# christopherkarani/Wax

Measured on NVIDIA H100. Metric: queries/sec cosine top-10 @ 10Mx384 fp32, higher is better.
Workload: dtype f32

## Files before the change

include/wax_vs_cuda.h:

```cpp
#ifndef WAX_VS_CUDA_H
#define WAX_VS_CUDA_H

#include <stddef.h>
#include <stdint.h>

#ifdef __cplusplus
extern "C" {
#endif

typedef struct wax_vs_engine wax_vs_engine;

enum {
    WAX_VS_OK = 0,
    WAX_VS_ERR_NULL = -1,
    WAX_VS_ERR_DIMENSION = -2,
    WAX_VS_ERR_CAPACITY = -3,
    WAX_VS_ERR_CUDA = -4,
    WAX_VS_ERR_FORMAT = -5,
    WAX_VS_ERR_ARGUMENT = -6,
    WAX_VS_ERR_BUFFER = -7,
    WAX_VS_ERR_UNSUPPORTED = -8
};

enum { WAX_VS_COSINE = 0, WAX_VS_DOT = 1, WAX_VS_L2 = 2 };
// ... 131 lines not shown
                             int64_t top_k, uint64_t row_offset, wax_vs_candidate *d_candidates,
                             void *cuda_stream);

int32_t wax_vs_search_batch_device(wax_vs_engine *engine, const float *d_queries, uint32_t n_queries,
                                   int64_t top_k, uint64_t row_offset, wax_vs_candidate *d_candidates,
                                   void *cuda_stream);

#define WAX_VS_SHARD_HANDLE_BYTES 128
#define WAX_VS_SHARD_MAX_RANKS 16
#define WAX_VS_SHARD_MAX_K 128
int32_t wax_vs_shard_open(wax_vs_engine *engine, int32_t rank, int32_t world, uint64_t row_offset,
                          uint8_t *out_handle );
int32_t wax_vs_shard_connect(wax_vs_engine *engine, const uint8_t *handles ,
                             int32_t n_handles);
int32_t wax_vs_shard_close(wax_vs_engine *engine);
int32_t wax_vs_shard_search(wax_vs_engine *engine, const float *query, uint32_t query_len, int64_t top_k,
                            uint64_t *out_ids, float *out_scores, uint32_t out_cap, uint32_t *out_n);
int32_t wax_vs_merge_candidates_device(wax_vs_engine *engine, const wax_vs_candidate *d_gathered, uint32_t world,
                                       uint32_t n_queries, uint32_t k, uint32_t k_out, wax_vs_candidate *d_out,
                                       void *cuda_stream);
int32_t wax_vs_shard_search_filtered(wax_vs_engine *engine, const float *query, uint32_t query_len, int64_t top_k,
                                     const uint64_t *frame_ids, uint64_t n_ids, int32_t mode, uint64_t *out_ids,
                                     float *out_scores, uint32_t out_cap, uint32_t *out_n);
int32_t wax_vs_shard_search_device(wax_vs_engine *engine, const float *d_query, int64_t top_k,
                                   wax_vs_candidate *d_candidates, void *cuda_stream);


int32_t wax_vs_serialized_length(wax_vs_engine *engine, uint64_t *out);
int32_t wax_vs_serialize(wax_vs_engine *engine, uint8_t *dst, uint64_t cap, uint64_t *out_len);
int32_t wax_vs_deserialize(wax_vs_engine *engine, const uint8_t *src, uint64_t len);

const char *wax_vs_last_error(void);


int32_t wax_vs_debug_pool_stats(wax_vs_engine *engine, uint64_t *allocations, uint64_t *reuses);

int32_t wax_vs_debug_fill_synthetic(wax_vs_engine *engine, uint64_t seed, uint64_t first_row,
                                    uint64_t rows, uint64_t id_base, int32_t normalize);
int32_t wax_vs_debug_read_rows(wax_vs_engine *engine, uint64_t first, uint64_t n, float *dst);

int32_t wax_vs_debug_time_search(wax_vs_engine *engine, uint32_t n_queries, int64_t top_k, uint64_t seed,
                                 uint32_t warmup, uint32_t iters, float *out_ms_total,
                                 uint64_t *out_launches);

int32_t wax_vs_debug_time_shard_search(wax_vs_engine *engine, uint32_t n_queries, int64_t top_k, uint64_t seed,
                                       uint32_t warmup, uint32_t iters, float *out_ms_total, uint64_t *out_launches);

int32_t wax_vs_debug_transfer_probe(wax_vs_engine *engine, uint64_t bytes, float *out7);

int32_t wax_vs_debug_phase_trace(wax_vs_engine *engine, int64_t top_k, uint32_t iters, float *out5);

int32_t wax_vs_debug_batch_stats(wax_vs_engine *engine, uint64_t *tensor_queries, uint64_t *fallback_queries);

int32_t wax_vs_debug_counter(wax_vs_engine *engine, const char *name, uint64_t *out);

int32_t wax_vs_debug_time_search_batch(wax_vs_engine *engine, uint32_t n_queries, int64_t top_k, uint64_t seed,
                                       uint32_t warmup, uint32_t iters, float *out_ms_total,
                                       uint64_t *out_launches, uint32_t *out_unproven);

int32_t wax_vs_debug_batch_nominations(wax_vs_engine *engine, const float *queries, uint32_t n_queries, int64_t top_k,
                                       const uint32_t *allow_bits, float *out_scores, uint32_t *out_ok,
                                       uint64_t *out_heaps, uint64_t heaps_cap, uint32_t *out_shape);

int32_t wax_vs_debug_shadow_nominations(wax_vs_engine *engine, const float *query, int64_t top_k, const uint32_t *allow_bits,
                                        uint64_t *out_keys, uint32_t *out_ok, wax_vs_candidate *out_result,
                                        uint32_t *out_shape);

int32_t wax_vs_debug_read_shadow(wax_vs_engine *engine, uint64_t first, uint64_t n, uint16_t *dst);

int32_t wax_vs_debug_int8_nominations(wax_vs_engine *engine, const float *query, int64_t top_k, const uint32_t *allow_bits,
                                      uint64_t *out_keys, uint32_t *out_ok, wax_vs_candidate *out_result,
                                      uint32_t *out_shape);

int32_t wax_vs_debug_read_int8_shadow(wax_vs_engine *engine, uint64_t first, uint64_t n, uint8_t *dst_codes,
                                      float *dst_scales, float *out_rho_max);

int32_t wax_vs_debug_u4_nominations(wax_vs_engine *engine, const float *query, int64_t top_k, const uint32_t *allow_bits,
                                    uint64_t *out_keys, uint64_t keys_cap, uint32_t *out_ok, wax_vs_candidate *out_result,
                                    uint32_t *out_shape, float *out_bound);

int32_t wax_vs_debug_read_u4_shadow(wax_vs_engine *engine, uint64_t first, uint64_t n, uint8_t *dst_codes,
                                    float *dst_half_steps, float *out_rho_max);

int32_t wax_vs_debug_stream_read(wax_vs_engine *engine, uint32_t iters, float *out_best_ms, uint64_t *out_bytes);

int32_t wax_vs_debug_set_option(wax_vs_engine *engine, const char *key, int64_t value);

const char *wax_vs_version(void);

#ifdef __cplusplus
}
#endif
#endif
```

wax_b200/_lib.py:

```python
from __future__ import annotations

import ctypes as C
from pathlib import Path

PKG = Path(__file__).resolve().parent
LIB_PATH = PKG / "libwaxvs_cuda.so"

OK, ERR_NULL, ERR_DIMENSION, ERR_CAPACITY, ERR_CUDA, ERR_FORMAT, ERR_ARGUMENT, ERR_BUFFER, ERR_UNSUPPORTED = (
    0, -1, -2, -3, -4, -5, -6, -7, -8)
MAX_RESULTS = 10_000
NO_FILTER = 0xFFFFFFFF
MAX_DIMENSIONS = 1_000_000
MAX_PER_GROUP = 128
SHARD_HANDLE_BYTES, SHARD_MAX_RANKS, SHARD_MAX_K = 128, 16, 128
INT64_MIN, INT64_MAX = -(1 << 63), (1 << 63) - 1


class Candidate(C.Structure):
    _fields_ = [("distance", C.c_float), ("valid", C.c_uint32), ("row", C.c_uint64), ("frame_id", C.c_uint64)]


class Where(C.Structure):
    _fields_ = [("after", C.c_int64), ("before", C.c_int64), ("all_tags", C.c_uint64), ("no_tags", C.c_uint64)]

# ... 18 lines not shown
    "wax_vs_remove": (C.c_int32, [_eng, C.c_uint64]),
    "wax_vs_remove_batch": (C.c_int32, [_eng, _u64p, C.c_uint64, _u64p]),
    "wax_vs_search": (C.c_int32, [_eng, _f32p, C.c_uint32, C.c_int64, _u64p, _f32p, C.c_uint32, _u32p]),
    "wax_vs_search_filtered": (C.c_int32, [_eng, _f32p, C.c_uint32, C.c_int64, _u64p, C.c_uint64, C.c_int32, _u64p, _f32p,
                                           C.c_uint32, _u32p]),
    "wax_vs_search_batch_filtered": (C.c_int32, [_eng, _f32p, C.c_uint32, C.c_uint32, C.c_int64, _u64p, C.c_uint64, C.c_int32,
                                                 _u64p, _f32p, C.c_uint32, _u32p]),
    "wax_vs_shard_search_filtered": (C.c_int32, [_eng, _f32p, C.c_uint32, C.c_int64, _u64p, C.c_uint64, C.c_int32, _u64p,
                                                 _f32p, C.c_uint32, _u32p]),
    "wax_vs_search_batch_multi_filtered": (C.c_int32, [_eng, _f32p, C.c_uint32, C.c_uint32, C.c_int64, _u64p, _u64p,
                                                       C.POINTER(C.c_int32), C.c_uint32, _u32p, _u64p, _f32p, C.c_uint32,
                                                       _u32p]),
    "wax_vs_set_groups": (C.c_int32, [_eng, _u64p, _u64p, C.c_uint64, _u64p]),
    "wax_vs_search_grouped": (C.c_int32, [_eng, _f32p, C.c_uint32, C.c_int64, C.c_uint32, _u64p, C.c_uint64, C.c_int32,
                                          _u64p, _f32p, _u64p, C.c_uint32, _u32p]),
    "wax_vs_search_batch_grouped": (C.c_int32, [_eng, _f32p, C.c_uint32, C.c_uint32, C.c_int64, C.c_uint32, _u64p,
                                                C.c_uint64, C.c_int32, _u64p, _f32p, _u64p, C.c_uint32, _u32p]),
    "wax_vs_set_attributes": (C.c_int32, [_eng, _u64p, C.POINTER(C.c_int64), _u64p, C.c_uint64, _u64p]),
    "wax_vs_search_batch_where": (C.c_int32, [_eng, _f32p, C.c_uint32, C.c_uint32, C.c_int64, _u64p, _u64p,
                                              C.POINTER(C.c_int32), C.c_uint32, _u32p, C.c_void_p, C.c_uint32, _u32p,
                                              _u64p, _f32p, C.c_uint32, _u32p]),
    "wax_vs_search_batch_grouped_where": (C.c_int32, [_eng, _f32p, C.c_uint32, C.c_uint32, C.c_int64, C.c_uint32, _u64p,
                                                      C.c_uint64, C.c_int32, C.c_void_p, _u64p, _f32p, _u64p, C.c_uint32,
                                                      _u32p]),
    "wax_vs_set_locations": (C.c_int32, [_eng, _u64p, _f64p, _f64p, C.c_uint64, _u64p]),
    "wax_vs_location_box": (C.c_int32, [C.c_double, C.c_double, C.c_double, C.POINTER(C.c_int32), C.POINTER(C.c_int32)]),
    "wax_vs_location_bin": (C.c_int32, [C.c_double, C.c_double, C.POINTER(C.c_int32), C.POINTER(C.c_int32)]),
    "wax_vs_search_batch_where_near": (C.c_int32, [_eng, _f32p, C.c_uint32, C.c_uint32, C.c_int64, _u64p, _u64p,
                                                   C.POINTER(C.c_int32), C.c_uint32, _u32p, C.c_void_p, C.c_uint32,
                                                   _u32p, _u64p, _f32p, C.c_uint32, _u32p]),
    "wax_vs_search_batch_grouped_where_near": (C.c_int32, [_eng, _f32p, C.c_uint32, C.c_uint32, C.c_int64, C.c_uint32,
                                                           _u64p, C.c_uint64, C.c_int32, C.c_void_p, _u64p, _f32p, _u64p,
                                                           C.c_uint32, _u32p]),
    "wax_vs_search_batch_grouped_multi_where": (C.c_int32, [_eng, _f32p, C.c_uint32, C.c_uint32, C.c_int64, C.c_uint32,
                                                            _u64p, _u64p, C.POINTER(C.c_int32), C.c_uint32, _u32p,
                                                            C.c_void_p, C.c_uint32, _u32p, _u64p, _f32p, _u64p,
                                                            C.c_uint32, _u32p]),
    "wax_vs_set_terms": (C.c_int32, [_eng, _u64p, _u64p, _u64p, C.c_uint64, _u64p]),
    "wax_vs_search_batch_where_terms": (C.c_int32, [_eng, _f32p, C.c_uint32, C.c_uint32, C.c_int64, _u64p, _u64p,
                                                    C.POINTER(C.c_int32), C.c_uint32, _u32p, C.c_void_p, C.c_uint32,
                                                    _u32p, _u64p, _u64p, _u64p, _f32p, C.c_uint32, _u32p]),
    "wax_vs_search_batch": (C.c_int32, [_eng, _f32p, C.c_uint32, C.c_uint32, C.c_int64, _u64p, _f32p,
                                        C.c_uint32, _u32p]),
    "wax_vs_search_device": (C.c_int32, [_eng, C.c_void_p, C.c_uint32, C.c_int64, C.c_uint64, C.c_void_p,
                                         C.c_void_p]),
    "wax_vs_search_batch_device": (C.c_int32, [_eng, C.c_void_p, C.c_uint32, C.c_int64, C.c_uint64, C.c_void_p,
                                               C.c_void_p]),
    "wax_vs_merge_candidates_device": (C.c_int32, [_eng, C.c_void_p, C.c_uint32, C.c_uint32, C.c_uint32, C.c_uint32,
                                                   C.c_void_p, C.c_void_p]),
    "wax_vs_shard_open": (C.c_int32, [_eng, C.c_int32, C.c_int32, C.c_uint64, _u8p]),
    "wax_vs_shard_connect": (C.c_int32, [_eng, _u8p, C.c_int32]),
    "wax_vs_shard_close": (C.c_int32, [_eng]),
    "wax_vs_shard_search": (C.c_int32, [_eng, _f32p, C.c_uint32, C.c_int64, _u64p, _f32p, C.c_uint32, _u32p]),
    "wax_vs_shard_search_device": (C.c_int32, [_eng, C.c_void_p, C.c_int64, C.c_void_p, C.c_void_p]),
    "wax_vs_serialized_length": (C.c_int32, [_eng, _u64p]),
    "wax_vs_serialize": (C.c_int32, [_eng, _u8p, C.c_uint64, _u64p]),
    "wax_vs_deserialize": (C.c_int32, [_eng, _u8p, C.c_uint64]),
    "wax_vs_last_error": (C.c_char_p, []),
    "wax_vs_debug_pool_stats": (C.c_int32, [_eng, _u64p, _u64p]),
    "wax_vs_debug_fill_synthetic": (C.c_int32, [_eng, C.c_uint64, C.c_uint64, C.c_uint64, C.c_uint64, C.c_int32]),
    "wax_vs_debug_read_rows": (C.c_int32, [_eng, C.c_uint64, C.c_uint64, _f32p]),
    "wax_vs_debug_time_search": (C.c_int32, [_eng, C.c_uint32, C.c_int64, C.c_uint64, C.c_uint32, C.c_uint32,
                                             _f32p, _u64p]),
    "wax_vs_debug_time_shard_search": (C.c_int32, [_eng, C.c_uint32, C.c_int64, C.c_uint64, C.c_uint32, C.c_uint32,
                                                   _f32p, _u64p]),
    "wax_vs_debug_transfer_probe": (C.c_int32, [_eng, C.c_uint64, _f32p]),
    "wax_vs_debug_phase_trace": (C.c_int32, [_eng, C.c_int64, C.c_uint32, _f32p]),
    "wax_vs_debug_batch_stats": (C.c_int32, [_eng, _u64p, _u64p]),
    "wax_vs_debug_counter": (C.c_int32, [_eng, C.c_char_p, _u64p]),
    "wax_vs_debug_time_search_batch": (C.c_int32, [_eng, C.c_uint32, C.c_int64, C.c_uint64, C.c_uint32, C.c_uint32,
                                                   _f32p, _u64p, _u32p]),
    "wax_vs_debug_batch_nominations": (C.c_int32, [_eng, _f32p, C.c_uint32, C.c_int64, _u32p, _f32p, _u32p, _u64p,
                                                   C.c_uint64, _u32p]),
    "wax_vs_debug_shadow_nominations": (C.c_int32, [_eng, _f32p, C.c_int64, _u32p, _u64p, _u32p, C.POINTER(Candidate),
                                                    _u32p]),
    "wax_vs_debug_read_shadow": (C.c_int32, [_eng, C.c_uint64, C.c_uint64, C.POINTER(C.c_uint16)]),
    "wax_vs_debug_int8_nominations": (C.c_int32, [_eng, _f32p, C.c_int64, _u32p, _u64p, _u32p, C.POINTER(Candidate),
                                                  _u32p]),
    "wax_vs_debug_read_int8_shadow": (C.c_int32, [_eng, C.c_uint64, C.c_uint64, _u8p, _f32p, _f32p]),
    "wax_vs_debug_u4_nominations": (C.c_int32, [_eng, _f32p, C.c_int64, _u32p, _u64p, C.c_uint64, _u32p,
                                                C.POINTER(Candidate), _u32p, _f32p]),
    "wax_vs_debug_read_u4_shadow": (C.c_int32, [_eng, C.c_uint64, C.c_uint64, _u8p, _f32p, _f32p]),
    "wax_vs_debug_stream_read": (C.c_int32, [_eng, C.c_uint32, _f32p, _u64p]),
    "wax_vs_debug_set_option": (C.c_int32, [_eng, C.c_char_p, C.c_int64]),
    "wax_vs_version": (C.c_char_p, []),
}

_lib = None


def lib() -> C.CDLL:
    global _lib
    if _lib is None:
        if not LIB_PATH.exists():
            raise ImportError(
                f"{LIB_PATH} is missing: the CUDA extension is the only implementation of the vector scan. "
                "Build it with `python -m wax_b200.build` (or __graft_entry__.build()).")
        handle = C.CDLL(str(LIB_PATH))
        for name, (restype, argtypes) in SIGNATURES.items():
            fn = getattr(handle, name)
            fn.restype = restype
            fn.argtypes = argtypes
        _lib = handle
    return _lib


def last_error() -> str:
    return lib().wax_vs_last_error().decode("utf-8", "replace")
```

wax_b200/csrc/waxvs_batch.cuh:

```cuda
#pragma once
#include <cuda.h>
#include <cuda_bf16.h>

#include "waxvs_common.cuh"
#include "waxvs_scan.cuh"

namespace waxvs {

constexpr int kBatchM = 128;
constexpr int kBatchN = 128;
constexpr int kBatchKBlock = 32;
constexpr int kBatchKBlockBf16 = 64;
constexpr int kBatchRescore = 256;
constexpr int kBatchRescoreMax = 1024;
constexpr uint32_t kBatchABytes = kBatchM * 128u;
constexpr uint32_t kBatchBBytes = kBatchN * 128u;
constexpr uint32_t kBatchStageBytes = kBatchABytes + kBatchBBytes;
constexpr int kBatchStageSlots = 8;
constexpr uint32_t kBatchScoreStride = kBatchN + 8;
constexpr uint32_t kBatchScoreBytes = kBatchM * kBatchScoreStride * 4u;
constexpr int kBatchMaxStages = 6;
constexpr uint32_t kBatchSmemOptin = 227u * 1024u;
__host__ __device__ constexpr uint32_t batch_smem_bytes(int stages, int heap, uint32_t ares_kb = 0) {
    return ares_kb * kBatchABytes + stages * (ares_kb ? kBatchBBytes : kBatchStageBytes) + kBatchScoreBytes +
// ... 141 lines not shown
                                                        float *inv_norm, uint32_t *max_norm_bits,
                                                        float *half_sq = nullptr) {
    const int lane = threadIdx.x & 31;
    const uint32_t warps = (gridDim.x * blockDim.x) >> 5;
    const bool vec4 = (dims % 4u) == 0u;
    float local_max = 0.0f;
    for (uint32_t row = (blockIdx.x * blockDim.x + threadIdx.x) >> 5; row < n_rows; row += warps) {
        const float *v = corpus + static_cast<size_t>(row) * dims;
        float b0 = 0.f, b1 = 0.f, b2 = 0.f, b3 = 0.f;
        if (vec4) {
            const float4 *v4 = reinterpret_cast<const float4 *>(v);
            for (uint32_t c = lane; c < dims / 4u; c += 32u) {
                const float4 x = __ldg(v4 + c);
                b0 = __fmaf_rn(x.x, x.x, b0); b1 = __fmaf_rn(x.y, x.y, b1);
                b2 = __fmaf_rn(x.z, x.z, b2); b3 = __fmaf_rn(x.w, x.w, b3);
            }
        } else {
            for (uint32_t base = 4u * lane; base < dims; base += 128u) {
                const float x = __ldg(v + base); b0 = __fmaf_rn(x, x, b0);
                if (base + 1 < dims) { const float y = __ldg(v + base + 1); b1 = __fmaf_rn(y, y, b1); }
                if (base + 2 < dims) { const float z = __ldg(v + base + 2); b2 = __fmaf_rn(z, z, b2); }
                if (base + 3 < dims) { const float w = __ldg(v + base + 3); b3 = __fmaf_rn(w, w, b3); }
            }
        }
        const float s = warp_butterfly_sum(__fadd_rn(__fadd_rn(b0, b1), __fadd_rn(b2, b3)));
        const float nrm = __fsqrt_rn(s);
        if (lane == 0) inv_norm[row] = (s == 0.0f) ? 0.0f : __fdiv_rn(1.0f, nrm);
        if constexpr (HALF_SQ) {
            if (lane == 0) half_sq[row] = 0.5f * s;
        }
        if (finite_f32(nrm)) {
            local_max = fmaxf(local_max, nrm);
        } else {
            float m = 0.0f;
            bool bad = false;
            for (uint32_t i = lane; i < dims; i += 32u) {
                const float x = __ldg(v + i);
                bad |= !finite_f32(x);
                m = fmaxf(m, fabsf(x));
            }
            if (!__any_sync(WAXVS_FULL_MASK, bad)) {
                for (int o = 16; o > 0; o >>= 1) m = fmaxf(m, __shfl_xor_sync(WAXVS_FULL_MASK, m, o));
                float t = 0.0f;
                for (uint32_t i = lane; i < dims; i += 32u) {
                    const float y = __fdiv_rn(__ldg(v + i), m);
                    t = __fmaf_rn(y, y, t);
                }
                local_max = fmaxf(local_max, m * __fsqrt_rn(warp_butterfly_sum(t)));
            }
        }
    }
    if (lane == 0 && local_max > 0.0f) atomicMax(max_norm_bits, __float_as_uint(local_max));
}

__global__ void __launch_bounds__(256) shadow_bf16_kernel(const float *__restrict__ src, const float *__restrict__ scale,
                                                          uint64_t n_rows, uint32_t dims, __nv_bfloat16 *__restrict__ dst) {
    const uint32_t d4 = dims >> 2;
    const uint64_t total = n_rows * d4;
    const float4 *s4 = reinterpret_cast<const float4 *>(src);
    uint2 *o = reinterpret_cast<uint2 *>(dst);
    for (uint64_t i = static_cast<uint64_t>(blockIdx.x) * blockDim.x + threadIdx.x; i < total;
         i += static_cast<uint64_t>(gridDim.x) * blockDim.x) {
        float4 x = __ldcs(s4 + i);
        if (scale) {
            const float w = __ldg(scale + i / d4);
            x.x *= w; x.y *= w; x.z *= w; x.w *= w;
        }
        const __nv_bfloat162 lo = __floats2bfloat162_rn(x.x, x.y), hi = __floats2bfloat162_rn(x.z, x.w);
        uint2 v;
        v.x = *reinterpret_cast<const uint32_t *>(&lo);
        v.y = *reinterpret_cast<const uint32_t *>(&hi);
        auto clamp_half = [](uint32_t h, float src) -> uint32_t {
            return ((h & 0x7FFFu) == 0x7F80u && finite_f32(src)) ? ((h & 0x8000u) | 0x7F7Fu) : h;
        };
        v.x = clamp_half(v.x & 0xFFFFu, x.x) | (clamp_half(v.x >> 16, x.y) << 16);
        v.y = clamp_half(v.y & 0xFFFFu, x.z) | (clamp_half(v.y >> 16, x.w) << 16);
        o[i] = v;
    }
}

constexpr uint32_t kInt8MaxChunks = 12;
__global__ void __launch_bounds__(256) shadow_int8_kernel(const float *__restrict__ src, const float *__restrict__ scale_in,
                                                          uint64_t n_rows, uint32_t dims, uint32_t *__restrict__ dst,
                                                          float *__restrict__ scale, uint32_t *rho_max_bits) {
    const int lane = threadIdx.x & 31;
    const uint64_t warps = (static_cast<uint64_t>(gridDim.x) * blockDim.x) >> 5;
    const uint32_t d4 = dims >> 2, cn = d4 / 32u;
    uint32_t local_max = 0;
    for (uint64_t row = (static_cast<uint64_t>(blockIdx.x) * blockDim.x + threadIdx.x) >> 5; row < n_rows; row += warps) {
        const float4 *v4 = reinterpret_cast<const float4 *>(src) + row * d4;
        const float w = scale_in ? __ldg(scale_in + row) : 1.0f;
        float4 x[kInt8MaxChunks];
        float m = 0.0f;
        bool bad = false;
#pragma unroll
        for (uint32_t c = 0; c < kInt8MaxChunks; ++c) {
            if (c >= cn) break;
            x[c] = __ldcs(v4 + lane + 32u * c);
            if (scale_in) { x[c].x *= w; x[c].y *= w; x[c].z *= w; x[c].w *= w; }
            bad |= !finite_f32(x[c].x) || !finite_f32(x[c].y) || !finite_f32(x[c].z) || !finite_f32(x[c].w);
            m = fmaxf(m, fmaxf(fmaxf(fabsf(x[c].x), fabsf(x[c].y)), fmaxf(fabsf(x[c].z), fabsf(x[c].w))));
        }
        for (int o = 16; o > 0; o >>= 1) m = fmaxf(m, __shfl_xor_sync(WAXVS_FULL_MASK, m, o));
        bad = __any_sync(WAXVS_FULL_MASK, bad);
        const float s = __fdiv_rn(m, 127.0f);
        double r2 = 0.0;
#pragma unroll
        for (uint32_t c = 0; c < kInt8MaxChunks; ++c) {
            if (c >= cn) break;
            const float xs[4] = {x[c].x, x[c].y, x[c].z, x[c].w};
            uint32_t packed = 0;
#pragma unroll
            for (int j = 0; j < 4; ++j) {
                int code = 0;
                if (s > 0.0f && !bad) code = max(-127, min(127, __float2int_rn(__fdiv_rn(xs[j], s))));
                packed |= static_cast<uint32_t>(code + 128) << (8 * j);
                const double e = static_cast<double>(xs[j]) - static_cast<double>(s) * static_cast<double>(code);
                r2 = fma(e, e, r2);
            }
            dst[row * d4 + lane + 32u * c] = packed;
        }
        for (int o = 16; o > 0; o >>= 1) r2 += __shfl_xor_sync(WAXVS_FULL_MASK, r2, o);
        float rho = __double2float_ru(sqrt(r2) * (1.0 + 0x1p-40));
        if (bad || !finite_f32(s) || !finite_f32(rho)) rho = INFINITY;
        if (lane == 0) scale[row] = s;
        local_max = max(local_max, __float_as_uint(rho));
    }
    if (lane == 0 && local_max) atomicMax(rho_max_bits, local_max);
}

__global__ void __launch_bounds__(256) shadow_u4_kernel(const float *__restrict__ src, const float *__restrict__ scale_in,
                                                        uint64_t n_rows, uint32_t dims, uint32_t *__restrict__ dst,
                                                        float *__restrict__ half_step, uint32_t *rho_max_bits) {
    const int lane = threadIdx.x & 31;
    const uint64_t warps = (static_cast<uint64_t>(gridDim.x) * blockDim.x) >> 5;
    const uint32_t d4 = dims >> 2, cn = d4 / 32u;
    uint32_t local_max = 0;
    for (uint64_t row = (static_cast<uint64_t>(blockIdx.x) * blockDim.x + threadIdx.x) >> 5; row < n_rows; row += warps) {
        const float4 *v4 = reinterpret_cast<const float4 *>(src) + row * d4;
        const float w = scale_in ? __ldg(scale_in + row) : 1.0f;
        float4 x[kInt8MaxChunks];
        float m = 0.0f;
        bool bad = false;
#pragma unroll
        for (uint32_t c = 0; c < kInt8MaxChunks; ++c) {
            if (c >= cn) break;
            x[c] = __ldcs(v4 + lane + 32u * c);
            if (scale_in) { x[c].x *= w; x[c].y *= w; x[c].z *= w; x[c].w *= w; }
            bad |= !finite_f32(x[c].x) || !finite_f32(x[c].y) || !finite_f32(x[c].z) || !finite_f32(x[c].w);
            m = fmaxf(m, fmaxf(fmaxf(fabsf(x[c].x), fabsf(x[c].y)), fmaxf(fabsf(x[c].z), fabsf(x[c].w))));
        }
        for (int o = 16; o > 0; o >>= 1) m = fmaxf(m, __shfl_xor_sync(WAXVS_FULL_MASK, m, o));
        bad = __any_sync(WAXVS_FULL_MASK, bad);
        const float h = __fdiv_rn(m, 16.0f), step = __fmul_rn(2.0f, h);
        double r2 = 0.0;
#pragma unroll
        for (uint32_t c = 0; c < kInt8MaxChunks; ++c) {
            if (c >= cn) break;
            const float xs[4] = {x[c].x, x[c].y, x[c].z, x[c].w};
            uint32_t nibbles = 0;
#pragma unroll
            for (int j = 0; j < 4; ++j) {
                int u = 8;
                if (h > 0.0f && !bad) u = max(0, min(15, __float2int_rd(__fdiv_rn(xs[j], step)) + 8));
                nibbles |= static_cast<uint32_t>(u) << (8 * j);
                const double e = static_cast<double>(xs[j]) - static_cast<double>(h) * static_cast<double>(2 * u - 15);
                r2 = fma(e, e, r2);
            }
            const uint32_t high = __shfl_down_sync(WAXVS_FULL_MASK, nibbles, 1);
            if ((lane & 1) == 0) dst[row * (d4 / 2u) + (lane >> 1) + 16u * c] = nibbles | (high << 4);
        }
        for (int o = 16; o > 0; o >>= 1) r2 += __shfl_xor_sync(WAXVS_FULL_MASK, r2, o);
        float rho = __double2float_ru(sqrt(r2) * (1.0 + 0x1p-40));
        if (bad || !finite_f32(h) || !finite_f32(rho)) rho = INFINITY;
        if (lane == 0) half_step[row] = h;
        local_max = max(local_max, __float_as_uint(rho));
    }
    if (lane == 0 && local_max) atomicMax(rho_max_bits, local_max);
}

template <bool BF16, bool FILTER, bool ARES, bool PAIR, bool DUMP = false, bool L2 = false>
__global__ void __launch_bounds__(kBatchThreads, 1)
batch_nominate_kernel(const __grid_constant__ CUtensorMap tmap_q, const __grid_constant__ CUtensorMap tmap_c,
                      const BatchParams p) {
    extern __shared__ uint8_t smem_raw[];
    uint8_t *smem = smem_raw + ((1024u - (smem_u32(smem_raw) & 1023u)) & 1023u);
    constexpr uint32_t KB_ELEMS = BF16 ? kBatchKBlockBf16 : kBatchKBlock;
    constexpr uint32_t STAGE_BYTES = ARES ? kBatchBBytes : kBatchStageBytes;
    constexpr uint32_t B_OFF = ARES ? 0u : kBatchABytes;
    const uint32_t num_kb = p.dims / KB_ELEMS;
    const uint32_t nst = p.stages, heap_n = p.kprime;
    const uint32_t ares_bytes = ARES ? num_kb * kBatchABytes : 0u;
    uint8_t *a_res = smem;
    uint8_t *stages = smem + ares_bytes;
    float *score = reinterpret_cast<float *>(stages + nst * STAGE_BYTES);
    float *scale_smem = score + kBatchM * kBatchScoreStride;
    uint64_t *full = reinterpret_cast<uint64_t *>(scale_smem + kBatchN);
    uint64_t *empty = full + kBatchMaxStages;
    uint64_t *a_full = empty + kBatchMaxStages;
    uint64_t *stage_smem = reinterpret_cast<uint64_t *>(reinterpret_cast<uint8_t *>(full) + 256);
    uint64_t *heap_smem = stage_smem + kBatchStageSlots * kBatchM;

    const int warp = threadIdx.x >> 5, lane = threadIdx.x & 31;
    const uint32_t rank = PAIR ? cluster_ctarank() : 0u;
    const uint32_t unit = PAIR ? blockIdx.x / 2u : blockIdx.x;
    const uint32_t units_per_slice = PAIR ? p.groups / 2u : p.groups;
    const uint32_t group = PAIR ? (unit % units_per_slice) * 2u + rank : unit % units_per_slice;
    const uint32_t slice = unit / units_per_slice;
    const uint32_t tile_lo = static_cast<uint32_t>(static_cast<uint64_t>(p.tiles_total) * slice / p.slices);
    const uint32_t tile_hi = static_cast<uint32_t>(static_cast<uint64_t>(p.tiles_total) * (slice + 1) / p.slices);

    if (warp == 4 && lane == 0) {
        tma_prefetch_desc(&tmap_q);
        tma_prefetch_desc(&tmap_c);
        for (int s = 0; s < kBatchMaxStages; ++s) { mbar_init(&full[s], 1); mbar_init(&empty[s], PAIR ? 8 : 4); }
        mbar_init(a_full, 1);
        mbar_fence_init();
    }
    if (PAIR) cluster_sync_all(); else __syncthreads();

    if (warp == 4) {
        if (lane == 0) {
            if (ARES && tile_lo < tile_hi) {
                mbar_arrive_expect_tx(a_full, ares_bytes);
                for (uint32_t kb = 0; kb < num_kb; ++kb)
                    tma_load_2d(a_res + kb * kBatchABytes, &tmap_q, a_full, static_cast<int32_t>(kb * KB_ELEMS),
                                static_cast<int32_t>(group * kBatchM));
            }
            uint32_t stage = 0, phase = 0;
            for (uint32_t tile = tile_lo; tile < tile_hi; ++tile) {
                for (uint32_t kb = 0; kb < num_kb; ++kb) {
                    mbar_wait_parity(&empty[stage], phase ^ 1u);
                    uint8_t *a = stages + stage * STAGE_BYTES;
                    mbar_arrive_expect_tx(&full[stage], STAGE_BYTES);
                    if (!ARES)
                        tma_load_2d(a, &tmap_q, &full[stage], static_cast<int32_t>(kb * KB_ELEMS), static_cast<int32_t>(group * kBatchM));
                    if (PAIR)
                        tma_load_2d_multicast(a + B_OFF + rank * (kBatchBBytes / 2), &tmap_c, &full[stage],
                                              static_cast<int32_t>(kb * KB_ELEMS),
                                              static_cast<int32_t>(tile * kBatchN + rank * (kBatchN / 2)), 0x3);
                    else
                        tma_load_2d(a + B_OFF, &tmap_c, &full[stage], static_cast<int32_t>(kb * KB_ELEMS),
                                    static_cast<int32_t>(tile * kBatchN));
                    if (++stage == nst) { stage = 0; phase ^= 1u; }
                }
            }
        }
        __syncwarp();
        if (PAIR) cluster_sync_all();
        return;
    }

    const uint32_t tid = threadIdx.x;
    const uint32_t q = group * kBatchM + tid;
    const bool q_valid = q < p.n_queries && !p.no_insert;
    const uint32_t *allow = p.allow_bits;
    if (p.query_filter && q < p.n_queries) {
        const uint32_t f = __ldg(p.query_filter + q);
// ... 694 lines not shown
```

wax_b200/csrc/waxvs_engine.cu:

```cuda
#include <cuda_runtime.h>

#include <algorithm>
#include <atomic>
#include <cstdarg>
#include <cstdio>
#include <cstring>
#include <mutex>
#include <new>
#include <shared_mutex>
#include <string>
#include <unordered_map>
#include <chrono>
#include <random>
#include <thread>
#include <unistd.h>
#include <cmath>
#include <vector>

#include "../../include/wax_vs_cuda.h"
#include "waxvs_common.cuh"
#include "waxvs_scan.cuh"
#include "waxvs_select.cuh"
#include "waxvs_synth.cuh"
#include "waxvs_batch.cuh"
// ... 132 lines not shown
    int batch_retry = 1;
    int filter_bf16 = 1;
    int filter_cap = 8192;
    int inline_query = 1;
    int host_delivery = 1;
    int tail_select = 1;
    int shard_fused = 1;
    int batch_l2 = 0;
    int single_shadow = 0;
    uint64_t filter_bitset_bytes = 2ull << 30;
    int shadow_scan = 1;
    uint64_t shadow_scan_min_bytes = 512ull << 20;
    int shadow_rows_per_step = 0, shadow_warps = 0, shadow_stages = 0;
    uint64_t int8_scan_min_bytes = 512ull << 20;
    int int8_rows_per_step = 0, int8_warps = 0, int8_stages = 0;
    uint64_t u4_scan_min_bytes = 2048ull << 20;
    int u4_rows_per_step = 0, u4_warps = 0, u4_stages = 0;
};

struct SearchCtx {
    cudaStream_t stream = nullptr;
    bool own_stream = false;
    DevBuf<float> d_queries;
    DevBuf<wax_vs_candidate> d_out;
    PinnedBuf<float> h_queries;
    PinnedBuf<wax_vs_candidate> h_out;
    DevBuf<uint64_t> d_block_keys;
    DevBuf<uint32_t> d_ticket;
    DevBuf<uint32_t> d_dist_keys;
    DevBuf<SelectState> d_select;
    DevBuf<uint64_t> d_sel_keys;
    cudaEvent_t ev0 = nullptr, ev1 = nullptr;
    DevBuf<uint64_t> d_heaps;
    DevBuf<uint32_t> d_ok;
    PinnedBuf<uint32_t> h_ok;
    DevBuf<uint32_t> d_tau;
    DevBuf<__nv_bfloat16> d_queries_bf16;
    DevBuf<float> d_retry_q;
    DevBuf<wax_vs_candidate> d_retry_out;
    DevBuf<uint32_t> d_retry_ok;
    DevBuf<float> d_tau_star;
    PinnedBuf<float> h_tau_star;
    DevBuf<float> d_filter_tau;
    PinnedBuf<float> h_filter_tau;
    DevBuf<uint32_t> d_cand_count;
    DevBuf<uint32_t> d_cand_rows;
    DevBuf<uint64_t> d_cand_keys;
    DevBuf<uint32_t> d_mask;
    DevBuf<uint32_t> d_filter_rows;
    DevBuf<uint64_t> d_filter_spec;
    DevBuf<uint32_t> d_query_filter;
    DevBuf<uint32_t> d_retry_filter;
    DevBuf<uint2> d_gather_span;
    DevBuf<uint64_t> d_gather_keys;
    DevBuf<wax_vs_candidate> d_shard_local;
    DevBuf<unsigned long long> d_group_best;
    DevBuf<uint32_t> d_group_keys;
    DevBuf<uint2> d_group_spans;
    PinnedBuf<uint2> h_group_spans;
    DevBuf<ExpandItem> d_expand_items;
    DevBuf<uint64_t> d_expand[3];
    PinnedBuf<uint64_t> h_expand;
    DevBuf<uint64_t> d_bg_keys;
    PinnedBuf<uint64_t> h_bg_keys;
    DevBuf<uint32_t> d_bg_status;
    PinnedBuf<uint32_t> h_bg_status;
    DevBuf<CoverExpand> d_bg_expand;
    PinnedBuf<CoverExpand> h_bg_expand;
    DevBuf<ScoreItem> d_score_items;
    PinnedBuf<unsigned long long> h_flag;
    unsigned long long host_seq = 0;
    DevBuf<WhereNearItem> d_where_items;
    DevBuf<uint32_t> d_where_counts;
    DevBuf<uint64_t> d_term_ids;
    DevBuf<TermSpan> d_term_spans;
    DevBuf<TermUnit> d_term_units;
    DevBuf<uint32_t> d_term_counts;
    DevBuf<uint32_t> d_term_deny;
    DevBuf<uint32_t> d_proof_count;
    PinnedBuf<uint32_t> h_proof_count;
    uint32_t seen_failed = 0;
    bool last_u4 = false;
    DevBuf<uint32_t> d_u4_aux;
    ~SearchCtx() {
        if (ev0) cudaEventDestroy(ev0);
        if (ev1) cudaEventDestroy(ev1);
        if (own_stream && stream) cudaStreamDestroy(stream);
    }
};

struct wax_vs_engine {
    int device = 0;
    int sm_count = 132;
    size_t smem_optin = 0;
    uint32_t dims = 0;
    uint8_t similarity = 0;

    float *d_corpus = nullptr;
    uint64_t cap_rows = 0, n_rows = 0;

    bool ids_identity = true;
    uint64_t id_base = 0;
    std::vector<uint64_t> ids;
    IdMap map;
    bool map_valid = true;
    bool ids_sorted = true;
    DevBuf<uint64_t> d_ids;
    bool d_ids_dirty = true;
    std::mutex ids_mu;

    std::shared_mutex rw;
    std::mutex pool_mu;
    std::vector<SearchCtx *> pool;
    std::unordered_map<void *, SearchCtx *> stream_ctx;
    uint64_t pool_allocs = 0, pool_reuses = 0;
    Tuning tune;

    DevBuf<float> d_inv_norm;
    DevBuf<uint32_t> d_max_norm;
    DevBuf<float> d_half_sq;
    uint64_t norms_rows = 0;
    std::mutex norms_mu;
    DevBuf<__nv_bfloat16> d_shadow;
    uint64_t shadow_rows = 0;
    bool shadow_valid = false, shadow_unavailable = false;
    struct CodedShadow {
        uint32_t bits = 8;
        DevBuf<uint32_t> codes;
        DevBuf<float> scale;
        DevBuf<uint32_t> rho;
        uint64_t rows = 0;
        bool valid = false, unavailable = false;
        bool coarse = false;
        float rho_max = 0.0f, eps_rel = INFINITY;
        void release() { codes.release(); scale.release(); rows = 0; valid = false; }
        void invalidate(uint64_t keep_prefix) {
            rows = std::min(rows, keep_prefix);
            valid = false;
            if (keep_prefix == 0) coarse = false;
        }
    } i8, u4{4};
    uint32_t u4_demoted = 0, u4_demote_window = 16;
    bool u4_probing = false;
    uint64_t single_int8_queries = 0;
    uint64_t single_u4_queries = 0;
    uint64_t batch_tensor_queries = 0, batch_fallback_queries = 0;
    uint64_t batch_bf16_queries = 0, batch_retry_queries = 0, batch_tf32_queries = 0, batch_filter_bf16_queries = 0;
    uint64_t filter_bitset_passes = 0;
    bool groups_set = false;
    std::vector<uint64_t> groups;
    struct GroupIndex {
        DevBuf<uint32_t> perm, row_group, starts;
        uint32_t n_groups = 0;
        bool valid = false;
    } gindex;
    std::mutex group_mu;
    uint64_t group_index_builds = 0;
    bool attrs_set = false;
    std::vector<AttrRow> attrs;
    DevBuf<AttrRow> d_attrs;
    bool attrs_dev_valid = false;
    std::mutex attrs_mu;
    uint64_t attribute_uploads = 0;
    bool locs_set = false;
    std::vector<LocRow> locs;
    DevBuf<LocRow> d_locs;
    bool locs_dev_valid = false;
    uint64_t location_uploads = 0;
    struct TermRef {
        uint64_t off;
        uint32_t n;
    };
    bool terms_set = false;
    std::vector<TermRef> term_refs;
    std::vector<uint64_t> term_pool;
    uint64_t term_garbage = 0;
    struct TermIndex {
        DevBuf<uint64_t> keys, start;
        DevBuf<uint32_t> postings;
        uint32_t n_terms = 0;
        uint64_t n_postings = 0;
        bool valid = false;
    } tindex;
    std::mutex term_mu;
    uint64_t term_index_builds = 0;
    uint64_t grouped_batch_covered_queries = 0, grouped_batch_expanded_groups = 0, grouped_batch_fallback_queries = 0;
    uint64_t grouped_batch_expansion_passes = 0;
    uint32_t bf16_skip_batches = 0;
    uint32_t shadow_scan_skip = 0;
    uint32_t heap_bump = 0, heap_bump_ttl = 0, heap_backoff = 256;
    bool heap_probing = false;
    uint32_t last_heap = 0;
    struct Ingest {
        cudaStream_t stream = nullptr;
        cudaEvent_t ev[2] = {nullptr, nullptr};
        uint8_t *pin[2] = {nullptr, nullptr};
        size_t pin_bytes = 0;
        DevBuf<float> d_stage;
        DevBuf<uint32_t> d_index;
        int threads = 1;
        ~Ingest() {
            for (int i = 0; i < 2; ++i) {
                if (pin[i]) cudaFreeHost(pin[i]);
                if (ev[i]) cudaEventDestroy(ev[i]);
            }
            if (stream) cudaStreamDestroy(stream);
        }
    } ing;
    uint64_t ingest_h2d_bytes = 0, ingest_d2h_bytes = 0;
    std::mutex ingest_mu;
    std::mutex attr_mu;
    std::unordered_map<const void *, int> smem_granted;
    std::atomic<bool> async_pending{false};
    unsigned long long *debug_trace = nullptr;

    struct Shard {
        bool open = false, connected = false;
        int rank = 0, world = 0;
// ... 329 lines not shown
    int32_t rc = c->d_select.ensure(1, "selection state");
    if (!rc) rc = c->d_sel_keys.ensure(16384, "selected keys");
    if (rc) return rc;
    const int sgrid = std::max(1, std::min<int>(e->sm_count * 4, static_cast<int>((n + 511) / 512)));
    select_init_kernel<<<1, 256, 0, stream>>>(c->d_select, k);
    for (int pass = 0; pass < kSelectPasses; ++pass) {
        select_hist_kernel<<<sgrid, 512, 0, stream>>>(keys, n, c->d_select, pass);
        select_scan_kernel<<<1, 1024, 0, stream>>>(c->d_select, pass);
    }
    select_compact_kernel<<<sgrid, 512, 0, stream>>>(keys, n, c->d_select, c->d_sel_keys, 16384);
    uint32_t pow2 = 64;
    while (pow2 < k) pow2 <<= 1;
    CUDA_TRY(grant_smem(e, select_sort_kernel, pow2 * sizeof(uint64_t)));
    select_sort_kernel<<<1, 1024, pow2 * sizeof(uint64_t), stream>>>(c->d_select, c->d_sel_keys, pow2, p);
    CUDA_TRY(cudaGetLastError());
    *launches += 3 + 2 * kSelectPasses;
    return WAX_VS_OK;
}

static int tma_grid(const wax_vs_engine *e, const SearchCtx *c, const TmaConfig &cfg, ScanParams &p) {
    p.stages = static_cast<uint32_t>(cfg.stages);
    const uint64_t steps = (e->n_rows + cfg.R - 1) / cfg.R;
    const int max_grid = e->tune.grid > 0 ? e->tune.grid : e->sm_count;
    int grid = static_cast<int>(std::min<uint64_t>(max_grid, (steps + cfg.warps - 1) / cfg.warps));
    grid = std::max(std::min(grid, static_cast<int>(c->d_block_keys.cap / 128)), 1);
    if (e->tune.chunk_steps < 0)
        p.chunk_steps = static_cast<uint32_t>(std::max<uint64_t>(1, std::min<uint64_t>(8, steps / (static_cast<uint64_t>(grid) * cfg.warps * 2))));
    return grid;
}

static bool batch_bf16_wanted(const wax_vs_engine *e);
static int32_t ensure_shadow(wax_vs_engine *e, cudaStream_t stream);
static int32_t ensure_coded_shadow(wax_vs_engine *e, wax_vs_engine::CodedShadow &cs, cudaStream_t stream, bool keep_coarse = false);

constexpr uint32_t kShadowNominees = 128;
constexpr uint32_t kShadowRescore = 256;
constexpr uint32_t kShadowSkipQueries = 16;
static bool shadow_route_applies(const wax_vs_engine *e) {
    return e->tune.shadow_scan && (e->similarity == WAX_VS_COSINE || e->similarity == WAX_VS_DOT) && !e->debug_trace &&
           e->tune.batch_bf16 != 0 && e->dims % kBatchKBlockBf16 == 0 &&
           e->n_rows * e->dims * sizeof(float) >= e->tune.shadow_scan_min_bytes;
}
static int32_t int8_route_selected(wax_vs_engine *e, cudaStream_t stream, bool *use) {
    *use = false;
    TmaConfig cfg{};
    if (e->n_rows * e->dims * sizeof(float) < e->tune.int8_scan_min_bytes || !pick_tma_config(e, &cfg, 1, 1)) return WAX_VS_OK;
    const int32_t rc = ensure_coded_shadow(e, e->i8, stream);
    if (rc) return rc;
    *use = e->i8.valid && e->i8.eps_rel <= kBf16Eps;
    return WAX_VS_OK;
}
enum class RouteForm { kBf16, kInt8, kU4 };
static int32_t select_route_form(wax_vs_engine *e, cudaStream_t stream, bool demoted, RouteForm *form) {
    *form = RouteForm::kBf16;
    TmaConfig cfg{};
    int32_t rc;
    if (!demoted && e->n_rows * e->dims * sizeof(float) >= e->tune.u4_scan_min_bytes && pick_u4_config(e, &cfg)) {
        if ((rc = ensure_coded_shadow(e, e->u4, stream))) return rc;
        if (e->u4.valid && std::isfinite(e->u4.eps_rel)) { *form = RouteForm::kU4; return WAX_VS_OK; }
    }
    bool int8 = false;
    if ((rc = int8_route_selected(e, stream, &int8))) return rc;
    if (int8) *form = RouteForm::kInt8;
    return WAX_VS_OK;
}

static int32_t enqueue_shadow_nominations(wax_vs_engine *e, SearchCtx *c, const ScanParams &p, const TmaConfig &cfg,
                                          cudaStream_t stream, uint64_t *launches, uint32_t *shape = nullptr,
                                          RouteForm form = RouteForm::kBf16) {
    const bool int8 = form == RouteForm::kInt8, u4 = form == RouteForm::kU4;
    int32_t rc;
    if (u4 && !c->d_u4_aux) {
        if ((rc = c->d_u4_aux.ensure(3, "4-bit route state"))) return rc;
        CUDA_TRY(cudaMemsetAsync(c->d_u4_aux, 0xFF, 3 * sizeof(uint32_t), stream));
    }
    const size_t u4_keys = static_cast<size_t>(std::max(e->tune.grid, e->sm_count)) * kU4CtaNominees;
    if ((rc = c->d_heaps.ensure(std::max(static_cast<size_t>(kShadowNominees) * kNomineeStride, u4 ? u4_keys : 0), "nominee keys")) ||
        (rc = c->d_ok.ensure(1, "proof flags")) || (!p.query && (rc = c->d_queries.ensure(e->dims, "query buffer"))))
        return rc;

    ScanParams sp = p;
    sp.corpus = u4 ? reinterpret_cast<const float *>(e->u4.codes.p)
                   : int8 ? reinterpret_cast<const float *>(e->i8.codes.p) : reinterpret_cast<const float *>(e->d_shadow.p);
    sp.row_scale = u4 ? e->u4.scale.p : int8 ? e->i8.scale.p : nullptr;
    sp.u4_aux = u4 ? c->d_u4_aux.p : nullptr;
    sp.k = kShadowNominees;
    sp.out = nullptr; sp.host_out = nullptr; sp.host_flag = nullptr;
    sp.nominees = c->d_heaps;
    sp.query_store = p.query ? nullptr : c->d_queries.p;
    sp.tail_select = e->tune.tail_select ? 1u : 0u;
    sp.tail_smem_bytes = static_cast<uint32_t>(static_cast<size_t>(cfg.warps) * cfg.stages * cfg.R * e->dims *
                                               (int8 ? 1 : sizeof(__nv_bfloat16)));
    const int grid = tma_grid(e, c, cfg, sp);
    if (u4) CUDA_TRY(launch_u4_scan(e, sp, grid, cfg, stream));
    else if (int8) CUDA_TRY(launch_int8_scan(e, sp, grid, cfg, e->similarity, stream));
    else CUDA_TRY(launch_shadow_scan(e, sp, grid, cfg, e->similarity, stream));

    if (u4) {
        RescoreParams rp{};
        rp.corpus = e->d_corpus; rp.query = p.query ? p.query : c->d_queries.p;
        rp.dims = e->dims; rp.k = p.k; rp.n_nominees = static_cast<uint32_t>(grid) * kU4CtaNominees;
        rp.nominees = c->d_heaps; rp.aux = c->d_u4_aux; rp.max_norm_bits = e->d_max_norm; rp.rho_max = e->u4.rho_max;
        rp.block_keys = c->d_block_keys; rp.ticket = c->d_ticket; rp.work_counter = sp.work_counter; rp.out = p.out; rp.ok = c->d_ok;
        rp.frame_ids = p.frame_ids; rp.id_base = p.id_base; rp.row_offset = p.row_offset;
        rp.tail_smem_bytes = static_cast<uint32_t>(grid) * p.k * sizeof(uint64_t);
        if (rp.tail_smem_bytes > 48u * 1024u) rp.tail_smem_bytes = 0;
        const auto kernel = e->similarity == WAX_VS_COSINE ? shadow_rescore_kernel<kCosine> : shadow_rescore_kernel<kDot>;
        kernel<<<grid, 512, rp.tail_smem_bytes, stream>>>(rp);
        CUDA_TRY(cudaGetLastError());
    } else {
    FinishParams fp{};
    fp.corpus = e->d_corpus; fp.queries = p.query ? p.query : c->d_queries.p;
    fp.n_rows = p.n_rows; fp.dims = e->dims; fp.n_queries = 1; fp.groups = 1; fp.slices = 1;
    fp.kprime = kShadowNominees; fp.k = p.k; fp.metric = e->similarity;
    fp.heaps = c->d_heaps; fp.max_norm_bits = e->d_max_norm;
    fp.out = p.out; fp.ok = c->d_ok;
    fp.frame_ids = p.frame_ids; fp.id_base = p.id_base; fp.row_offset = p.row_offset;
    fp.pow2_all = 512; fp.rescore = kShadowRescore; fp.eps_rel = int8 ? e->i8.eps_rel : kBf16Eps;
    const size_t fsmem = static_cast<size_t>(fp.pow2_all + fp.rescore) * sizeof(uint64_t);
    const auto kernel = e->similarity == WAX_VS_COSINE ? batch_finish_kernel<kCosine> : batch_finish_kernel<kDot>;
    CUDA_TRY(grant_smem(e, kernel, fsmem));
    kernel<<<1, 512, fsmem, stream>>>(fp);
    CUDA_TRY(cudaGetLastError());
    }
    *launches += 2;
    if (shape) {
        const uint32_t s[7] = {static_cast<uint32_t>(cfg.C), static_cast<uint32_t>(cfg.R), static_cast<uint32_t>(cfg.warps),
                               static_cast<uint32_t>(cfg.stages), static_cast<uint32_t>(grid), sp.chunk_steps, sp.tail_select};
        std::copy(s, s + 7, shape);
    }
    return WAX_VS_OK;
}

static int32_t enqueue_shadow_route(wax_vs_engine *e, SearchCtx *c, ScanParams &p, cudaStream_t stream, uint64_t *launches) {
    if (!shadow_route_applies(e)) return WAX_VS_OK;
    TmaConfig cfg{};
    if (!pick_tma_config(e, &cfg, 1, sizeof(__nv_bfloat16))) return WAX_VS_OK;
    int32_t rc;
    if (!c->h_proof_count) {
        if ((rc = c->d_proof_count.ensure(2, "proof counts")) || (rc = c->h_proof_count.ensure(2, "proof count mirror"))) return rc;
        CUDA_TRY(cudaMemsetAsync(c->d_proof_count, 0, 2 * sizeof(uint32_t), stream));
        c->h_proof_count[0] = c->h_proof_count[1] = 0;
        c->seen_failed = 0;
    }
    bool demoted;
    {
        std::lock_guard<std::mutex> pg(e->pool_mu);
        const uint32_t failed = *static_cast<volatile uint32_t *>(c->h_proof_count + 1);
        if (failed != c->seen_failed) {
            c->seen_failed = failed;
            if (c->last_u4) {
                if (e->u4_probing) e->u4_demote_window = std::min(e->u4_demote_window * 2, 1u << 20);
                e->u4_demoted = e->u4_demote_window;
            } else {
                e->shadow_scan_skip = kShadowSkipQueries;
            }
        } else if (c->last_u4 && e->u4_probing) {
            e->u4_demote_window = 16;
        }
        if (c->last_u4) e->u4_probing = false;
        c->last_u4 = false;
        if (e->shadow_scan_skip > 0) { --e->shadow_scan_skip; return WAX_VS_OK; }
        demoted = e->u4_demoted > 0;
        if (demoted && --e->u4_demoted == 0) e->u4_probing = true;
    }
    RouteForm form;
    if ((rc = select_route_form(e, stream, demoted, &form))) return rc;
    if (form == RouteForm::kU4) {
        if (!pick_u4_config(e, &cfg)) return WAX_VS_OK;
    } else if (form == RouteForm::kInt8) {
        if (!pick_tma_config(e, &cfg, 1, 1)) return WAX_VS_OK;
    } else {
        if ((rc = ensure_shadow(e, stream))) return rc;
        if (!e->shadow_valid) return WAX_VS_OK;
    }
    if ((rc = enqueue_shadow_nominations(e, c, p, cfg, stream, launches, nullptr, form))) return rc;
    c->last_u4 = form == RouteForm::kU4;
    if (form != RouteForm::kBf16) {
        std::lock_guard<std::mutex> pg(e->pool_mu);
        ++(form == RouteForm::kU4 ? e->single_u4_queries : e->single_int8_queries);
    }
    p.proof_ok = c->d_ok;
    p.proof_count = c->d_proof_count;
    p.proof_count_host = c->h_proof_count;
    return WAX_VS_OK;
}

static ScanParams scan_params(const wax_vs_engine *e, SearchCtx *c, const float *d_query, uint32_t k_eff, uint64_t row_offset,
                              wax_vs_candidate *d_out, const uint64_t *d_ids, const uint32_t *d_mask) {
    ScanParams p{};
    p.corpus = e->d_corpus; p.query = d_query;
    p.n_rows = static_cast<uint32_t>(e->n_rows); p.dims = e->dims; p.k = k_eff;
// ... 153 lines not shown
        e->norms_rows = 0;
        const size_t want = static_cast<size_t>(std::max<uint64_t>(e->cap_rows, std::max<uint64_t>(e->n_rows, 1)));
        int32_t rc = e->d_inv_norm.ensure(want, "row norms");
        if (!rc && l2) rc = e->d_half_sq.ensure(want, "row half squared norms");
        if (rc) return rc;
    }
    if (!e->d_max_norm) {
        int32_t rc = e->d_max_norm.ensure(1, "max row norm");
        if (rc) return rc;
        e->norms_rows = 0;
    }
    if (e->norms_rows > e->n_rows) e->norms_rows = 0;
    if (e->norms_rows == 0) CUDA_TRY(cudaMemsetAsync(e->d_max_norm, 0, sizeof(uint32_t), stream));
    const uint64_t first = e->norms_rows, count = e->n_rows - first;
    if (count) {
        const int grid = static_cast<int>(std::min<uint64_t>(static_cast<uint64_t>(e->sm_count) * 8, (count + 7) / 8));
        if (l2)
            row_norms_kernel<true><<<std::max(grid, 1), 256, 0, stream>>>(e->d_corpus + first * e->dims, static_cast<uint32_t>(count),
                                                                          e->dims, e->d_inv_norm + first, e->d_max_norm,
                                                                          e->d_half_sq + first);
        else
            row_norms_kernel<<<std::max(grid, 1), 256, 0, stream>>>(e->d_corpus + first * e->dims, static_cast<uint32_t>(count), e->dims,
                                                                    e->d_inv_norm + first, e->d_max_norm);
        CUDA_TRY(cudaGetLastError());
    }
    CUDA_TRY(cudaStreamSynchronize(stream));
    e->norms_rows = e->n_rows;
    return WAX_VS_OK;
}
static int32_t ensure_norms(wax_vs_engine *e, cudaStream_t stream) {
    std::lock_guard<std::mutex> g(e->norms_mu);
    return ensure_norms_locked(e, stream);
}

static bool batch_bf16_wanted(const wax_vs_engine *e) {
    return e->tune.batch_bf16 != 0 && e->dims % kBatchKBlockBf16 == 0 && !e->shadow_unavailable;
}

static int32_t ensure_shadow(wax_vs_engine *e, cudaStream_t stream) {
    std::lock_guard<std::mutex> g(e->norms_mu);
    if ((e->shadow_valid && e->shadow_rows == e->n_rows) || e->shadow_unavailable) return WAX_VS_OK;
    int32_t rc = ensure_norms_locked(e, stream);
    if (rc) return rc;
    const size_t need = static_cast<size_t>(e->n_rows) * e->dims;
    const size_t pref = static_cast<size_t>(std::max<uint64_t>(e->cap_rows, e->n_rows)) * e->dims;
    if (e->d_shadow.cap < need) {
        e->d_shadow.release();
        e->shadow_rows = 0; e->shadow_valid = false;
        size_t free_b = 0, total_b = 0;
        size_t want = pref;
        size_t bytes = want * sizeof(__nv_bfloat16);
        const bool info = cudaMemGetInfo(&free_b, &total_b) == cudaSuccess;
        const size_t headroom = std::max<size_t>(size_t(2) << 30, total_b / 10);
        if (info && free_b < bytes + headroom) { want = need; bytes = want * sizeof(__nv_bfloat16); }
        if (!info || free_b < bytes + headroom || cudaMalloc(&e->d_shadow.p, bytes) != cudaSuccess) {
            cudaGetLastError();
            e->shadow_unavailable = true;
            return WAX_VS_OK;
        }
        e->d_shadow.cap = want;
    }
    if (e->shadow_rows > e->n_rows) e->shadow_rows = 0;
    const uint64_t first = e->shadow_rows, count = e->n_rows - first;
    if (count) {
        const int grid = static_cast<int>(std::min<uint64_t>(static_cast<uint64_t>(e->sm_count) * 16, (count * (e->dims / 4) + 255) / 256));
        shadow_bf16_kernel<<<std::max(grid, 1), 256, 0, stream>>>(e->d_corpus + first * e->dims,
                                                                  e->similarity == WAX_VS_COSINE ? e->d_inv_norm + first : nullptr,
                                                                  count, e->dims, e->d_shadow + first * e->dims);
        CUDA_TRY(cudaGetLastError());
    }
    CUDA_TRY(cudaStreamSynchronize(stream));
    e->shadow_rows = e->n_rows;
    e->shadow_valid = true;
    return WAX_VS_OK;
}

static int32_t ensure_coded_shadow(wax_vs_engine *e, wax_vs_engine::CodedShadow &cs, cudaStream_t stream, bool keep_coarse) {
    std::lock_guard<std::mutex> g(e->norms_mu);
    if ((cs.valid && cs.rows == e->n_rows) || cs.unavailable || (cs.coarse && !keep_coarse))
        return WAX_VS_OK;
    int32_t rc = ensure_norms_locked(e, stream);
    if (rc) return rc;
    if ((rc = cs.rho.ensure(1, "coded shadow bound"))) return rc;
    const size_t words = e->dims * cs.bits / 32;
    const uint64_t need = e->n_rows, pref = std::max<uint64_t>(e->cap_rows, e->n_rows);
    auto scale_entries = [](uint64_t rows) { return static_cast<size_t>((rows + 15) / 16 * 16); };
    if (cs.codes.cap < need * words || cs.scale.cap < scale_entries(need)) {
        cs.release();
        size_t free_b = 0, total_b = 0;
        uint64_t want = pref;
        auto bytes_for = [&](uint64_t rows) { return rows * words * sizeof(uint32_t) + scale_entries(rows) * sizeof(float); };
        const bool info = cudaMemGetInfo(&free_b, &total_b) == cudaSuccess;
        const size_t headroom = std::max<size_t>(size_t(2) << 30, total_b / 10);
        size_t reserve = 0;
        if (batch_bf16_wanted(e) && e->d_shadow.cap < static_cast<size_t>(need) * e->dims) {
            const size_t b_need = static_cast<size_t>(need) * e->dims * sizeof(__nv_bfloat16);
            const size_t b_pref = static_cast<size_t>(pref) * e->dims * sizeof(__nv_bfloat16);
            reserve = free_b >= b_pref + headroom ? b_pref : (free_b >= b_need + headroom ? b_need : 0);
        }
        if (info && free_b < bytes_for(want) + reserve + headroom) want = need;
        if (!info || free_b < bytes_for(want) + reserve + headroom ||
            cudaMalloc(&cs.codes.p, want * words * sizeof(uint32_t)) != cudaSuccess ||
            cudaMalloc(&cs.scale.p, scale_entries(want) * sizeof(float)) != cudaSuccess) {
            cudaGetLastError();
            cs.release();
            cs.unavailable = true;
            return WAX_VS_OK;
        }
        cs.codes.cap = want * words;
        cs.scale.cap = scale_entries(want);
        CUDA_TRY(cudaMemsetAsync(cs.scale, 0, scale_entries(want) * sizeof(float), stream));
    }
    if (cs.rows > e->n_rows) cs.rows = 0;
    if (cs.rows == 0) CUDA_TRY(cudaMemsetAsync(cs.rho, 0, sizeof(uint32_t), stream));
    const uint64_t first = cs.rows, count = e->n_rows - first;
    if (count) {
        const int grid = static_cast<int>(std::min<uint64_t>(static_cast<uint64_t>(e->sm_count) * 8, (count + 7) / 8));
        (cs.bits == 4 ? shadow_u4_kernel : shadow_int8_kernel)<<<std::max(grid, 1), 256, 0, stream>>>(
            e->d_corpus + first * e->dims, e->similarity == WAX_VS_COSINE ? e->d_inv_norm + first : nullptr, count, e->dims,
            cs.codes + first * words, cs.scale + first, cs.rho);
        CUDA_TRY(cudaGetLastError());
    }
    uint32_t bits[2] = {0, 0};
    CUDA_TRY(cudaMemcpyAsync(&bits[0], cs.rho, sizeof(uint32_t), cudaMemcpyDeviceToHost, stream));
    CUDA_TRY(cudaMemcpyAsync(&bits[1], e->d_max_norm, sizeof(uint32_t), cudaMemcpyDeviceToHost, stream));
    CUDA_TRY(cudaStreamSynchronize(stream));
    float rho, m;
    memcpy(&rho, &bits[0], sizeof rho);
    memcpy(&m, &bits[1], sizeof m);
    if (e->similarity == WAX_VS_COSINE) m = 1.0f;
    const float q = rho / m;
    cs.rho_max = rho;
    cs.eps_rel = (std::isfinite(q) && std::isfinite(m) && m > 0.0f)
                          ? (static_cast<double>(q) * m >= rho ? q : std::nextafter(q, INFINITY)) : INFINITY;
    cs.rows = e->n_rows;
    cs.valid = true;
    if (cs.bits == 4 ? !std::isfinite(cs.eps_rel) : cs.eps_rel > kBf16Eps) {
        cs.coarse = true;
        if (!keep_coarse) {
            cs.release();
        }
    }
    return WAX_VS_OK;
}

template <bool BF, bool FI, bool AR, bool PR, bool DUMP, bool L2>
static cudaError_t launch_nominate_inst(wax_vs_engine *e, uint32_t grid, uint32_t smem, cudaStream_t stream,
                                        const CUtensorMap &map_q, const CUtensorMap &map_c, const BatchParams &bp) {
    const auto kernel = batch_nominate_kernel<BF, FI, AR, PR, DUMP, L2>;
    const cudaError_t err = grant_smem(e, kernel, smem);
    if (err != cudaSuccess) return err;
    cudaLaunchConfig_t cfg{};
    cfg.gridDim = dim3(grid); cfg.blockDim = dim3(kBatchThreads); cfg.stream = stream; cfg.dynamicSmemBytes = smem;
    cudaLaunchAttribute attr[1];
    if (PR) {
        attr[0].id = cudaLaunchAttributeClusterDimension;
        attr[0].val.clusterDim.x = 2; attr[0].val.clusterDim.y = 1; attr[0].val.clusterDim.z = 1;
        cfg.attrs = attr; cfg.numAttrs = 1;
    }
    return cudaLaunchKernelEx(&cfg, kernel, map_q, map_c, bp);
}

template <bool DUMP, bool L2>
static cudaError_t launch_nominate_forms(wax_vs_engine *e, bool bf16, bool filter, bool ares, bool pair, uint32_t grid,
                                         uint32_t smem, cudaStream_t stream, const CUtensorMap &map_q,
                                         const CUtensorMap &map_c, const BatchParams &bp) {
#define WAXVS_NOM(BF, FI, AR, PR) return launch_nominate_inst<BF, FI, AR, PR, DUMP, L2>(e, grid, smem, stream, map_q, map_c, bp)
    if constexpr (!DUMP) {
        if (filter) {
            if (!bf16) WAXVS_NOM(false, true, false, false);
            if (ares) WAXVS_NOM(true, true, true, false);
            WAXVS_NOM(true, true, false, false);
        }
    }
    if (!bf16) {
        if (pair) WAXVS_NOM(false, false, false, true);
        WAXVS_NOM(false, false, false, false);
    }
    if (ares) {
        if (pair) WAXVS_NOM(true, false, true, true);
        WAXVS_NOM(true, false, true, false);
    }
    if (pair) WAXVS_NOM(true, false, false, true);
    WAXVS_NOM(true, false, false, false);
#undef WAXVS_NOM
}
template <bool DUMP>
static cudaError_t launch_nominate(wax_vs_engine *e, bool l2, bool bf16, bool filter, bool ares, bool pair, uint32_t grid,
                                   uint32_t smem, cudaStream_t stream, const CUtensorMap &map_q, const CUtensorMap &map_c,
                                   const BatchParams &bp) {
    return l2 ? launch_nominate_forms<DUMP, true>(e, bf16, filter, ares, pair, grid, smem, stream, map_q, map_c, bp)
              : launch_nominate_forms<DUMP, false>(e, bf16, filter, ares, pair, grid, smem, stream, map_q, map_c, bp);
}

static double poisson_tail(double m, int h) {
    double term = std::exp(-m);
    for (int i = 1; i <= h; ++i) term *= m / i;
    double tail = 0.0, t = term;
    for (int i = h + 1; i < h + 200 && t > 1e-300; ++i) { tail += t; t *= m / i; }
    return std::min(1.0, tail + t);
}

static uint32_t pick_heap(wax_vs_engine *e, bool bf16, uint32_t nq, uint32_t slices, uint32_t k_eff) {
// ... 2993 lines not shown
}

int32_t wax_vs_debug_time_search(wax_vs_engine *e, uint32_t n_queries, int64_t top_k, uint64_t seed,
                                 uint32_t warmup, uint32_t iters, float *out_ms_total, uint64_t *out_launches) {
    if (!e || !out_ms_total) return fail(WAX_VS_ERR_NULL, "NULL argument");
    if (n_queries == 0) n_queries = 1;
    std::shared_lock<std::shared_mutex> r(e->rw);
    DeviceGuard g(e->device);
    CtxLease lease(e);
    int32_t rc = lease.acquire();
    if (rc) return rc;
    SearchCtx *c = lease.c;
    const uint32_t k_eff = clamp_topk(top_k);
    const size_t qfloats = static_cast<size_t>(n_queries) * e->dims;
    if ((rc = c->d_queries.ensure(qfloats, "query buffer"))) return rc;
    if ((rc = c->d_out.ensure(static_cast<size_t>(n_queries) * k_eff, "result buffer"))) return rc;
    synth_fill_kernel<<<(n_queries + 255) / 256, 256, 0, c->stream>>>(c->d_queries, n_queries, e->dims, seed, 0, 1);
    CUDA_TRY(cudaGetLastError());
    uint64_t launches = 0;
    CtxLease lease2(e);
    if (e->tune.time_overlap) {
        if ((rc = lease2.acquire())) return rc;
        if ((rc = lease2.c->d_out.ensure(static_cast<size_t>(n_queries) * k_eff, "result buffer"))) return rc;
    }
    SearchCtx *c2 = lease2.c;
    if (shadow_route_applies(e)) {
        RouteForm form;
        if ((rc = select_route_form(e, c->stream, false, &form))) return rc;
        if (form == RouteForm::kBf16 && (rc = ensure_shadow(e, c->stream))) return rc;
    }
    for (uint32_t it = 0; it < warmup + iters; ++it) {
        if (it == warmup) {
            launches = 0;
            if (c2) { CUDA_TRY(cudaEventRecord(c2->ev0, c2->stream)); CUDA_TRY(cudaStreamWaitEvent(c->stream, c2->ev0, 0)); }
            CUDA_TRY(cudaEventRecord(c->ev0, c->stream));
            if (c2) CUDA_TRY(cudaStreamWaitEvent(c2->stream, c->ev0, 0));
        }
        const uint32_t qi = it % n_queries;
        SearchCtx *cc = (c2 && (it & 1u)) ? c2 : c;
        if (c2 && it == 0) { CUDA_TRY(cudaEventRecord(c->ev1, c->stream)); CUDA_TRY(cudaStreamWaitEvent(c2->stream, c->ev1, 0)); }
        rc = enqueue_search(e, cc, c->d_queries + static_cast<size_t>(qi) * e->dims, k_eff, 0,
                            cc->d_out + static_cast<size_t>(qi) * k_eff, nullptr, cc->stream, &launches, nullptr, nullptr,
                            nullptr, false, true);
        if (rc) { cudaStreamSynchronize(c->stream); if (c2) cudaStreamSynchronize(c2->stream); return rc; }
    }
    if (c2) { CUDA_TRY(cudaEventRecord(c2->ev1, c2->stream)); CUDA_TRY(cudaStreamWaitEvent(c->stream, c2->ev1, 0)); }
    CUDA_TRY(cudaEventRecord(c->ev1, c->stream));
    CUDA_TRY(cudaStreamSynchronize(c->stream));
    CUDA_TRY(cudaEventElapsedTime(out_ms_total, c->ev0, c->ev1));
    if (out_launches) *out_launches = launches;
    return WAX_VS_OK;
}

int32_t wax_vs_debug_stream_read(wax_vs_engine *e, uint32_t iters, float *out_best_ms, uint64_t *out_bytes) {
    if (!e || !out_best_ms || !out_bytes) return fail(WAX_VS_ERR_NULL, "NULL argument");
    std::shared_lock<std::shared_mutex> r(e->rw);
    DeviceGuard g(e->device);
    CtxLease lease(e);
    int32_t rc = lease.acquire();
    if (rc) return rc;
    SearchCtx *c = lease.c;
    const uint64_t bytes = e->n_rows * e->dims * sizeof(float) / 16 * 16;
    *out_bytes = bytes;
    *out_best_ms = 0.0f;
    if (bytes == 0) return WAX_VS_OK;
    float best = 1e30f;
    for (uint32_t it = 0; it < iters + 2; ++it) {
        CUDA_TRY(cudaEventRecord(c->ev0, c->stream));
        stream_read_kernel<<<e->sm_count * 4, 512, 0, c->stream>>>(reinterpret_cast<const uint4 *>(e->d_corpus),
                                                                     bytes / 16, c->d_ticket + 2);
        CUDA_TRY(cudaGetLastError());
        CUDA_TRY(cudaEventRecord(c->ev1, c->stream));
        CUDA_TRY(cudaStreamSynchronize(c->stream));
        float ms = 0;
        CUDA_TRY(cudaEventElapsedTime(&ms, c->ev0, c->ev1));
        if (it >= 2 && ms < best) best = ms;
    }
    CUDA_TRY(cudaMemsetAsync(c->d_ticket, 0, 4 * sizeof(uint32_t), c->stream));
    CUDA_TRY(cudaStreamSynchronize(c->stream));
    *out_best_ms = best;
    return WAX_VS_OK;
}

int32_t wax_vs_debug_transfer_probe(wax_vs_engine *e, uint64_t bytes, float *out7) {
    if (!e || !out7) return fail(WAX_VS_ERR_NULL, "NULL argument");
    std::unique_lock<std::shared_mutex> w(e->rw);
    DeviceGuard g(e->device);
    bytes = std::max<uint64_t>(bytes, 1u << 20);
    int32_t rc = ingest_staging(e, bytes);
    if (rc) return rc;
    auto &ig = e->ing;
    if ((rc = ig.d_stage.ensure(static_cast<size_t>((bytes + 3) / 4), "probe buffer"))) return rc;
    std::vector<uint8_t> host(bytes, 1);
    auto secs = [](auto t0) { return std::chrono::duration<double>(std::chrono::steady_clock::now() - t0).count(); };
    uint8_t *probe_pin = nullptr;
    {
        std::lock_guard<std::mutex> pool(g_staging_mu);
        if ((rc = shared_staging())) return rc;
        probe_pin = g_staging[0];
    }
    const size_t chunk = std::min<size_t>(kStagingBytes, bytes);
    auto best = [&](auto fn) { double b = 1e30; for (int i = 0; i < 3; ++i) { auto t0 = std::chrono::steady_clock::now(); fn(); b = std::min(b, secs(t0)); } return b; };
    out7[0] = static_cast<float>(chunk / 1e9 / best([&] { memcpy(probe_pin, host.data(), chunk); }));
    out7[1] = static_cast<float>(chunk / 1e9 / best([&] { parallel_memcpy(probe_pin, host.data(), chunk, ig.threads); }));
    out7[2] = static_cast<float>(chunk / 1e9 / best([&] { cudaMemcpyAsync(ig.d_stage, probe_pin, chunk, cudaMemcpyHostToDevice, ig.stream); cudaStreamSynchronize(ig.stream); }));
    out7[3] = static_cast<float>(chunk / 1e9 / best([&] { cudaMemcpyAsync(probe_pin, ig.d_stage, chunk, cudaMemcpyDeviceToHost, ig.stream); cudaStreamSynchronize(ig.stream); }));
    out7[4] = static_cast<float>(bytes / 1e9 / best([&] { upload_bytes(e, ig.d_stage, host.data(), bytes); }));
    out7[5] = static_cast<float>(bytes / 1e9 / best([&] { download_bytes(e, host.data(), ig.d_stage, bytes); }));
    out7[6] = static_cast<float>(ig.threads);
    CUDA_TRY(cudaGetLastError());
    return WAX_VS_OK;
}

int32_t wax_vs_debug_phase_trace(wax_vs_engine *e, int64_t top_k, uint32_t iters, float *out5) {
    if (!e || !out5) return fail(WAX_VS_ERR_NULL, "NULL argument");
    std::unique_lock<std::shared_mutex> w(e->rw);
    DeviceGuard g(e->device);
    CtxLease lease(e, true);
    int32_t rc = lease.acquire();
    if (rc) return rc;
    SearchCtx *c = lease.c;
    const uint32_t k_eff = clamp_topk(top_k);
    if ((rc = c->d_queries.ensure(static_cast<size_t>(e->dims), "query buffer"))) return rc;
    if ((rc = c->d_out.ensure(static_cast<size_t>(k_eff), "result buffer"))) return rc;
    synth_fill_kernel<<<1, 256, 0, c->stream>>>(c->d_queries, 1, e->dims, 99, 0, 1);
    unsigned long long *d_trace = nullptr;
    CUDA_TRY(cudaMalloc(&d_trace, 8 * sizeof(unsigned long long)));
    double acc[5] = {0, 0, 0, 0, 0};
    uint64_t launches = 0;
    for (uint32_t it = 0; it < iters + 3; ++it) {
        const unsigned long long init[8] = {~0ull, 0, 0, 0, 0, 0, 0, 0};
        cudaMemcpyAsync(d_trace, init, sizeof init, cudaMemcpyHostToDevice, c->stream);
        cudaStreamSynchronize(c->stream);
        e->debug_trace = d_trace;
        cudaEventRecord(c->ev0, c->stream);
        rc = enqueue_search(e, c, c->d_queries, k_eff, 0, c->d_out, nullptr, c->stream, &launches);
        cudaEventRecord(c->ev1, c->stream);
        e->debug_trace = nullptr;
        if (rc) { cudaStreamSynchronize(c->stream); cudaFree(d_trace); return rc; }
        unsigned long long t[8];
        cudaMemcpyAsync(t, d_trace, sizeof t, cudaMemcpyDeviceToHost, c->stream);
        cudaStreamSynchronize(c->stream);
        float ms = 0;
        cudaEventElapsedTime(&ms, c->ev0, c->ev1);
        if (it < 3) continue;
        for (int i = 0; i < 4; ++i) acc[i] += (t[i + 1] > t[0] && t[0] != ~0ull) ? (t[i + 1] - t[0]) * 1e-3 : 0.0;
        acc[4] += ms * 1e3;
    }
    cudaFree(d_trace);
    for (int i = 0; i < 5; ++i) out5[i] = static_cast<float>(acc[i] / std::max(iters, 1u));
    CUDA_TRY(cudaGetLastError());
    return WAX_VS_OK;
}

int32_t wax_vs_debug_batch_stats(wax_vs_engine *e, uint64_t *tensor_queries, uint64_t *fallback_queries) {
    if (!e) return fail(WAX_VS_ERR_NULL, "engine is NULL");
    std::lock_guard<std::mutex> g(e->pool_mu);
    if (tensor_queries) *tensor_queries = e->batch_tensor_queries;
    if (fallback_queries) *fallback_queries = e->batch_fallback_queries;
    return WAX_VS_OK;
}

int32_t wax_vs_debug_counter(wax_vs_engine *e, const char *name, uint64_t *out) {
    if (!e || !name || !out) return fail(WAX_VS_ERR_NULL, "NULL argument");
    std::lock_guard<std::mutex> g(e->pool_mu);
    if (!strcmp(name, "batch_tensor_queries")) *out = e->batch_tensor_queries;
// ... 142 lines not shown
                                       uint32_t *out_shape, RouteForm form, uint64_t keys_cap = 0, float *out_bound = nullptr) {
    const bool u4 = form == RouteForm::kU4, int8 = form != RouteForm::kBf16;
    if (!e || !query || !out_keys || !out_ok || !out_result || !out_shape || (u4 && !out_bound))
        return fail(WAX_VS_ERR_NULL, "NULL argument");
    std::shared_lock<std::shared_mutex> r(e->rw);
    const uint32_t k_eff = static_cast<uint32_t>(std::min<uint64_t>(clamp_topk(top_k), std::max<uint64_t>(e->n_rows, 1)));
    TmaConfig cfg{};
    if (e->n_rows == 0 || k_eff > 32u || (e->similarity != WAX_VS_COSINE && e->similarity != WAX_VS_DOT) ||
        (int8 ? (e->tune.batch_bf16 == 0 || e->dims % kBatchKBlockBf16 != 0) : !batch_bf16_wanted(e)) ||
        !(u4 ? pick_u4_config(e, &cfg) : pick_tma_config(e, &cfg, 1, int8 ? 1 : sizeof(__nv_bfloat16))))
        return fail(WAX_VS_ERR_UNSUPPORTED, "no %s-shadow route for k=%u, dims=%u in this shape",
                    u4 ? "4-bit" : int8 ? "int8" : "bf16", k_eff, e->dims);
    DeviceGuard g(e->device);
    if (!g.ok) return g.error();
    CtxLease lease(e);
    int32_t rc = lease.acquire();
    if (rc) return rc;
    SearchCtx *c = lease.c;
    if (int8) {
        wax_vs_engine::CodedShadow &cs = u4 ? e->u4 : e->i8;
        if ((rc = ensure_coded_shadow(e, cs, c->stream, true))) return rc;
        if (!cs.valid) return fail(WAX_VS_ERR_UNSUPPORTED, "the coded shadow does not fit in device memory");
    } else {
        if ((rc = ensure_shadow(e, c->stream))) return rc;
        if (!e->shadow_valid) return fail(WAX_VS_ERR_UNSUPPORTED, "the bf16 shadow does not fit in device memory");
    }
    if ((rc = c->d_out.ensure(k_eff, "result buffer"))) return rc;
    const uint32_t *d_mask = nullptr;
    if (allow_bits) {
        const size_t words = static_cast<size_t>((e->n_rows + 31) / 32);
        if ((rc = c->d_mask.ensure(words, "row filter"))) return rc;
        CUDA_TRY(cudaMemcpyAsync(c->d_mask, allow_bits, words * sizeof(uint32_t), cudaMemcpyHostToDevice, c->stream));
        d_mask = c->d_mask;
    }
    ScanParams p = scan_params(e, c, nullptr, k_eff, 0, c->d_out, nullptr, d_mask);
    if ((rc = place_host_query(e, c, p, query, true, c->stream))) return rc;
    uint64_t launches = 0;
    if ((rc = enqueue_shadow_nominations(e, c, p, cfg, c->stream, &launches, out_shape, form))) {
        cudaStreamSynchronize(c->stream);
        return rc;
    }
    CUDA_TRY(cudaStreamSynchronize(c->stream));
    if (u4) {
        const uint64_t n_keys = static_cast<uint64_t>(out_shape[4]) * kU4CtaNominees;
        if (keys_cap < n_keys)
            return fail(WAX_VS_ERR_BUFFER, "the nominees need %llu entries (%llu given)", static_cast<unsigned long long>(n_keys),
                        static_cast<unsigned long long>(keys_cap));
        CUDA_TRY(cudaMemcpy(out_keys, c->d_heaps, n_keys * sizeof(uint64_t), cudaMemcpyDeviceToHost));
        uint32_t aux[3];
        CUDA_TRY(cudaMemcpy(aux, c->d_u4_aux, sizeof aux, cudaMemcpyDeviceToHost));
        out_bound[0] = e->u4.rho_max;
        memcpy(out_bound + 1, &aux[1], sizeof(float));
        if (aux[2] == 0xFFFFFFFFu) out_bound[2] = -INFINITY;
        else { const uint32_t u = aux[2] ^ ((aux[2] & 0x80000000u) ? 0x80000000u : 0xFFFFFFFFu); float f; memcpy(&f, &u, 4); out_bound[2] = -f; }
    } else
    CUDA_TRY(cudaMemcpy2D(out_keys, sizeof(uint64_t), c->d_heaps, kNomineeStride * sizeof(uint64_t), sizeof(uint64_t),
                          kShadowNominees, cudaMemcpyDeviceToHost));
    CUDA_TRY(cudaMemcpy(out_ok, c->d_ok, sizeof(uint32_t), cudaMemcpyDeviceToHost));
    CUDA_TRY(cudaMemcpy(out_result, c->d_out, k_eff * sizeof(wax_vs_candidate), cudaMemcpyDeviceToHost));
    for (uint32_t i = 0; i < k_eff; ++i)
        if (out_result[i].valid) out_result[i].frame_id = frame_id_of(e, out_result[i].row);
    return WAX_VS_OK;
}

int32_t wax_vs_debug_shadow_nominations(wax_vs_engine *e, const float *query, int64_t top_k, const uint32_t *allow_bits,
                                        uint64_t *out_keys, uint32_t *out_ok, wax_vs_candidate *out_result,
                                        uint32_t *out_shape) {
    return debug_route_nominations(e, query, top_k, allow_bits, out_keys, out_ok, out_result, out_shape, RouteForm::kBf16);
}

int32_t wax_vs_debug_int8_nominations(wax_vs_engine *e, const float *query, int64_t top_k, const uint32_t *allow_bits,
                                      uint64_t *out_keys, uint32_t *out_ok, wax_vs_candidate *out_result,
                                      uint32_t *out_shape) {
    return debug_route_nominations(e, query, top_k, allow_bits, out_keys, out_ok, out_result, out_shape, RouteForm::kInt8);
}

int32_t wax_vs_debug_u4_nominations(wax_vs_engine *e, const float *query, int64_t top_k, const uint32_t *allow_bits,
                                    uint64_t *out_keys, uint64_t keys_cap, uint32_t *out_ok, wax_vs_candidate *out_result,
                                    uint32_t *out_shape, float *out_bound) {
    return debug_route_nominations(e, query, top_k, allow_bits, out_keys, out_ok, out_result, out_shape, RouteForm::kU4,
                                   keys_cap, out_bound);
}

int32_t wax_vs_debug_read_u4_shadow(wax_vs_engine *e, uint64_t first, uint64_t n, uint8_t *dst_codes, float *dst_half_steps,
                                    float *out_rho_max) {
    if (!e || !dst_codes || !dst_half_steps || !out_rho_max) return fail(WAX_VS_ERR_NULL, "NULL argument");
    std::shared_lock<std::shared_mutex> r(e->rw);
    if (first > e->n_rows || n > e->n_rows - first) return fail(WAX_VS_ERR_ARGUMENT, "row range out of bounds");
    TmaConfig cfg{};
    if ((e->similarity != WAX_VS_COSINE && e->similarity != WAX_VS_DOT) || !pick_u4_config(e, &cfg))
        return fail(WAX_VS_ERR_UNSUPPORTED, "no 4-bit shadow for dims=%u with this metric", e->dims);
    DeviceGuard g(e->device);
    if (!g.ok) return g.error();
    CtxLease lease(e);
    int32_t rc = lease.acquire();
    if (rc) return rc;
    if ((rc = ensure_coded_shadow(e, e->u4, lease.c->stream, true))) return rc;
    if (!e->u4.valid) return fail(WAX_VS_ERR_UNSUPPORTED, "the 4-bit shadow does not fit in device memory");
    if (n) {
        CUDA_TRY(cudaMemcpy(dst_codes, e->u4.codes + first * (e->dims / 8), n * e->dims / 2, cudaMemcpyDeviceToHost));
        CUDA_TRY(cudaMemcpy(dst_half_steps, e->u4.scale + first, n * sizeof(float), cudaMemcpyDeviceToHost));
    }
    *out_rho_max = e->u4.rho_max;
    return WAX_VS_OK;
}

int32_t wax_vs_debug_read_int8_shadow(wax_vs_engine *e, uint64_t first, uint64_t n, uint8_t *dst_codes, float *dst_scales,
                                      float *out_rho_max) {
    if (!e || !dst_codes || !dst_scales || !out_rho_max) return fail(WAX_VS_ERR_NULL, "NULL argument");
    std::shared_lock<std::shared_mutex> r(e->rw);
    if (first > e->n_rows || n > e->n_rows - first) return fail(WAX_VS_ERR_ARGUMENT, "row range out of bounds");
    TmaConfig cfg{};
    if ((e->similarity != WAX_VS_COSINE && e->similarity != WAX_VS_DOT) || !pick_tma_config(e, &cfg, 1, 1))
        return fail(WAX_VS_ERR_UNSUPPORTED, "no int8 shadow for dims=%u with this metric", e->dims);
    DeviceGuard g(e->device);
    if (!g.ok) return g.error();
    CtxLease lease(e);
    int32_t rc = lease.acquire();
    if (rc) return rc;
    if ((rc = ensure_coded_shadow(e, e->i8, lease.c->stream, true))) return rc;
    if (!e->i8.valid) return fail(WAX_VS_ERR_UNSUPPORTED, "the int8 shadow does not fit in device memory");
    if (n) {
        CUDA_TRY(cudaMemcpy(dst_codes, e->i8.codes + first * (e->dims / 4), n * e->dims, cudaMemcpyDeviceToHost));
        CUDA_TRY(cudaMemcpy(dst_scales, e->i8.scale + first, n * sizeof(float), cudaMemcpyDeviceToHost));
    }
    *out_rho_max = e->i8.rho_max;
    return WAX_VS_OK;
}

int32_t wax_vs_debug_read_shadow(wax_vs_engine *e, uint64_t first, uint64_t n, uint16_t *dst) {
    if (!e || !dst) return fail(WAX_VS_ERR_NULL, "NULL argument");
    std::shared_lock<std::shared_mutex> r(e->rw);
    if (first > e->n_rows || n > e->n_rows - first) return fail(WAX_VS_ERR_ARGUMENT, "row range out of bounds");
    if (!batch_bf16_wanted(e)) return fail(WAX_VS_ERR_UNSUPPORTED, "no bf16 shadow for dims=%u with these options", e->dims);
    DeviceGuard g(e->device);
    if (!g.ok) return g.error();
    CtxLease lease(e);
    int32_t rc = lease.acquire();
    if (rc) return rc;
    if ((rc = ensure_shadow(e, lease.c->stream))) return rc;
    if (!e->shadow_valid) return fail(WAX_VS_ERR_UNSUPPORTED, "the bf16 shadow does not fit in device memory");
    if (n) CUDA_TRY(cudaMemcpy(dst, e->d_shadow + first * e->dims, n * e->dims * sizeof(__nv_bfloat16), cudaMemcpyDeviceToHost));
    return WAX_VS_OK;
}

int32_t wax_vs_debug_set_option(wax_vs_engine *e, const char *key, int64_t value) {
    if (!e || !key) return fail(WAX_VS_ERR_NULL, "NULL argument");
    std::unique_lock<std::shared_mutex> w(e->rw);
    const int v = static_cast<int>(value);
    if (!strcmp(key, "variant")) e->tune.variant = v;
    else if (!strcmp(key, "rows_per_step")) e->tune.rows_per_step = v;
    else if (!strcmp(key, "stages")) e->tune.stages = v;
    else if (!strcmp(key, "warps")) e->tune.warps = v;
    else if (!strcmp(key, "grid")) e->tune.grid = v;
    else if (!strcmp(key, "l2_hint")) e->tune.l2_hint = v;
    else if (!strcmp(key, "chunk_steps")) e->tune.chunk_steps = v;
    else if (!strcmp(key, "fused_k_max")) e->tune.fused_k_max = std::max(0, std::min(128, v));
    else if (!strcmp(key, "batch_tensor")) e->tune.batch_tensor = v;
    else if (!strcmp(key, "batch_min")) e->tune.batch_min = v;
    else if (!strcmp(key, "batch_noinsert")) e->tune.batch_noinsert = v;
    else if (!strcmp(key, "batch_heap")) e->tune.batch_heap = v;
    else if (!strcmp(key, "batch_large_k")) e->tune.batch_large_k = v;
    else if (!strcmp(key, "tma_max_dims")) e->tune.tma_max_dims = static_cast<uint32_t>(std::max(v, 0));
    else if (!strcmp(key, "batch_pair")) e->tune.batch_pair = v;
    else if (!strcmp(key, "batch_ares")) e->tune.batch_ares = v;
    else if (!strcmp(key, "batch_bf16")) { e->tune.batch_bf16 = v; e->shadow_unavailable = false; e->bf16_skip_batches = 0; }
    else if (!strcmp(key, "batch_rescore")) e->tune.batch_rescore = v;
    else if (!strcmp(key, "batch_retry")) e->tune.batch_retry = v;
    else if (!strcmp(key, "filter_cap")) e->tune.filter_cap = v;
    else if (!strcmp(key, "filter_bf16")) e->tune.filter_bf16 = v;
    else if (!strcmp(key, "batch_l2")) e->tune.batch_l2 = v;
    else if (!strcmp(key, "filter_bitset_bytes")) e->tune.filter_bitset_bytes = static_cast<uint64_t>(std::max<int64_t>(value, 0));
    else if (!strcmp(key, "single_shadow")) e->tune.single_shadow = v;
    else if (!strcmp(key, "shadow_scan")) {
        std::lock_guard<std::mutex> pg(e->pool_mu);
        e->tune.shadow_scan = v;
        e->shadow_scan_skip = 0;
        auto seen = [](SearchCtx *c) { if (c->h_proof_count) c->seen_failed = *static_cast<volatile uint32_t *>(c->h_proof_count + 1); };
        for (SearchCtx *c : e->pool) seen(c);
        for (auto &kv : e->stream_ctx) seen(kv.second);
    }
    else if (!strcmp(key, "shadow_rows_per_step")) e->tune.shadow_rows_per_step = v;
    else if (!strcmp(key, "shadow_warps")) e->tune.shadow_warps = v;
    else if (!strcmp(key, "shadow_stages")) e->tune.shadow_stages = v;
    else if (!strcmp(key, "shadow_scan_min_bytes")) e->tune.shadow_scan_min_bytes = static_cast<uint64_t>(std::max<int64_t>(value, 0));
    else if (!strcmp(key, "int8_scan_min_bytes")) {
        e->tune.int8_scan_min_bytes = static_cast<uint64_t>(std::max<int64_t>(value, 0));
        e->i8.unavailable = false;
        e->i8.coarse = false;
    }
    else if (!strcmp(key, "u4_scan_min_bytes")) {
        e->tune.u4_scan_min_bytes = static_cast<uint64_t>(std::max<int64_t>(value, 0));
        e->u4.unavailable = false;
        e->u4.coarse = false;
        e->u4_demoted = 0; e->u4_demote_window = 16; e->u4_probing = false;
    }
    else if (!strcmp(key, "u4_rows_per_step")) e->tune.u4_rows_per_step = v;
    else if (!strcmp(key, "u4_warps")) e->tune.u4_warps = v;
    else if (!strcmp(key, "u4_stages")) e->tune.u4_stages = v;
    else if (!strcmp(key, "int8_rows_per_step")) e->tune.int8_rows_per_step = v;
    else if (!strcmp(key, "int8_warps")) e->tune.int8_warps = v;
    else if (!strcmp(key, "int8_stages")) e->tune.int8_stages = v;
    else if (!strcmp(key, "shard_fused")) e->tune.shard_fused = v;
    else if (!strcmp(key, "tail_select")) e->tune.tail_select = v;
    else if (!strcmp(key, "inline_query")) e->tune.inline_query = v;
    else if (!strcmp(key, "host_delivery")) e->tune.host_delivery = v;
    else if (!strcmp(key, "shard_timeout_ms")) e->shard.timeout_ns = static_cast<unsigned long long>(std::max<int64_t>(value, 1)) * 1000000ull;
// ... 8 lines not shown
```

wax_b200/csrc/waxvs_scan.cuh:

```cuda
#pragma once
#include "waxvs_common.cuh"
#include "waxvs_shard.cuh"
#include "../../include/wax_vs_cuda.h"

namespace waxvs {

constexpr int kInlineQueryFloats = 512;

struct ScanParams {
    const float *corpus;
    const float *query;
    uint32_t n_rows;
    uint32_t dims;
    uint32_t k;
    uint32_t stages;
    uint64_t *block_keys;
    uint32_t *ticket;
    wax_vs_candidate *out;
    uint32_t *dist_keys;
    const uint64_t *frame_ids;
    uint64_t id_base;
    uint64_t row_offset;
    uint32_t use_l2_hint;
    uint32_t chunk_steps;
    uint32_t *work_counter;
    const uint32_t *mask;
    wax_vs_candidate *host_out;
    unsigned long long *host_flag;
    unsigned long long host_seq;
    alignas(16) float query_inline[kInlineQueryFloats];
    uint32_t tail_select;
    uint32_t tail_smem_bytes;
    unsigned long long *trace;
    ShardParams shard;
    uint64_t *nominees;
    float *query_store;
    const uint32_t *proof_ok;
    uint32_t *proof_count;
    uint32_t *proof_count_host;
    const float *row_scale;
    uint32_t *u4_aux;
};

constexpr uint32_t kU4CtaNominees = 256;

constexpr int kNomineeStride = 128;

__device__ __forceinline__ bool row_allowed(const ScanParams &p, uint32_t row) {
    return p.mask == nullptr || ((__ldg(p.mask + (row >> 5)) >> (row & 31u)) & 1u) != 0u;
}

__device__ __forceinline__ void write_candidate(const ScanParams &p, int slot, uint64_t key) {
    wax_vs_candidate c;
    if (key == WAXVS_KEY_NONE) {
        c.distance = 0.0f; c.valid = 0; c.row = 0; c.frame_id = 0;
    } else {
        const uint32_t row = static_cast<uint32_t>(key);
        c.distance = from_orderable_u32(static_cast<uint32_t>(key >> 32));
        c.valid = 1;
        c.row = p.row_offset + row;
        c.frame_id = p.frame_ids ? p.frame_ids[row] : p.id_base + row;
    }
    p.out[slot] = c;
    if (p.host_out) p.host_out[slot] = c;
}

template <bool SHADOW>
__device__ __forceinline__ void write_slot(const ScanParams &p, int slot, uint64_t key) {
    if constexpr (SHADOW) p.nominees[static_cast<size_t>(slot == static_cast<int>(p.k) - 1 ? 0 : slot + 1) * kNomineeStride] = key;
    else write_candidate(p, slot, key);
}

__device__ __forceinline__ float4 bf16x4_to_float4(uint2 u) {
    return make_float4(__uint_as_float(u.x << 16), __uint_as_float(u.x & 0xFFFF0000u),
                       __uint_as_float(u.y << 16), __uint_as_float(u.y & 0xFFFF0000u));
}

__device__ __forceinline__ float4 int8x4_to_float4(uint32_t u) {
    constexpr float kBias = 8388736.0f;
    return make_float4(__fsub_rn(__uint_as_float(__byte_perm(u, 0x4B000000u, 0x7650)), kBias),
                       __fsub_rn(__uint_as_float(__byte_perm(u, 0x4B000000u, 0x7651)), kBias),
                       __fsub_rn(__uint_as_float(__byte_perm(u, 0x4B000000u, 0x7652)), kBias),
                       __fsub_rn(__uint_as_float(__byte_perm(u, 0x4B000000u, 0x7653)), kBias));
}

template <int H>
__device__ __forceinline__ void half_warp_reduce_scatter(int (&v)[H], int lane) {
    static_assert(H == 1 || H == 2 || H == 4 || H == 8, "H must be a power of two <= 8");
    int off = 8;
#pragma unroll
    for (int half = H / 2; half >= 1; half >>= 1, off >>= 1) {
        const bool upper = (lane & off) != 0;
#pragma unroll
        for (int j = 0; j < half; ++j) {
            const int send = upper ? v[j] : v[j + half];
            const int keep = upper ? v[j + half] : v[j];
            v[j] = keep + __shfl_xor_sync(WAXVS_FULL_MASK, send, off);
        }
    }
#pragma unroll
    for (; off >= 1; off >>= 1) v[0] += __shfl_xor_sync(WAXVS_FULL_MASK, v[0], off);
}

template <int E, bool SHADOW = false>
__device__ __forceinline__ void finish_topk(const ScanParams &p, WarpTopK<E> &tk, uint64_t *lists, int warp,
                                            int lane, int warps) {
    const int k = static_cast<int>(p.k);
    constexpr int W = E * 32;
    __shared__ uint32_t s_last;
    auto load_list = [&](const uint64_t *src, uint64_t (&dst)[E]) {
#pragma unroll
        for (int j = 0; j < E; ++j) dst[j] = src[j * 32 + lane];
    };
#pragma unroll
    for (int j = 0; j < E; ++j) lists[warp * W + j * 32 + lane] = tk.key[j];
    __syncthreads();
    if (warp == 0) {
#pragma unroll 1
        for (int w = 1; w < warps; ++w) {
            uint64_t other[E];
            load_list(lists + w * W, other);
            tk.merge_sorted(other, lane, k);
        }
#pragma unroll
        for (int j = 0; j < E; ++j) p.block_keys[static_cast<size_t>(blockIdx.x) * W + j * 32 + lane] = tk.key[j];
        __threadfence();
        __syncwarp();
// ... 113 lines not shown
    uint64_t *mine = p.block_keys + static_cast<size_t>(blockIdx.x) * k;
#pragma unroll
    for (int j = 0; j < E; ++j)
        if (tk.key[j] != WAXVS_KEY_NONE && tk.key[j] <= xa) mine[atomicAdd(&ss.n_sel, 1u)] = tk.key[j];
    __syncthreads();
    for (uint32_t i = ss.n_sel + tid; i < k; i += nthr) mine[i] = WAXVS_KEY_NONE;
    __threadfence();
    __syncthreads();
    if (p.trace && tid == 0) atomicMax(p.trace + 2, global_timer_ns());
    if (tid == 0) s_last2 = (atomicAdd(p.ticket, 1u) == gridDim.x - 1) ? 1u : 0u;
    __syncthreads();
    if (!s_last2) return false;
    __threadfence();
    if (p.trace && tid == 0) p.trace[3] = global_timer_ns();
    const uint32_t total = gridDim.x * k;
    const bool staged = static_cast<size_t>(total) * sizeof(uint64_t) <= p.tail_smem_bytes;
    uint64_t *sk = reinterpret_cast<uint64_t *>(scratch);
    if (staged) {
        for (uint32_t i = tid; i < total; i += nthr) sk[i] = ld_cg_u64(p.block_keys + i);
        __syncthreads();
    }
    auto grid_keys = [&](auto f) {
        if (staged) { for (uint32_t i = tid; i < total; i += nthr) f(sk[i]); }
        else { for (uint32_t i = tid; i < total; i += nthr) f(ld_cg_u64(p.block_keys + i)); }
    };
    const uint64_t xb = block_select_kth(grid_keys, k, &ss);
    if (tid == 0) ss.n_sel = 0;
    __syncthreads();
    grid_keys([&](uint64_t key) { if (key != WAXVS_KEY_NONE && key <= xb) ss.sel[atomicAdd(&ss.n_sel, 1u)] = key; });
    __syncthreads();
    const uint32_t n_sel = ss.n_sel;
    for (uint32_t i = tid; i < k; i += nthr) {
        if (i < n_sel) {
            const uint64_t key = ss.sel[i];
            uint32_t rank = 0;
            for (uint32_t j = 0; j < n_sel; ++j) rank += ss.sel[j] < key ? 1u : 0u;
            write_slot<SHADOW>(p, static_cast<int>(rank), key);
        } else {
            write_slot<SHADOW>(p, static_cast<int>(i), WAXVS_KEY_NONE);
        }
    }
    if (p.host_flag && !p.shard.world) __threadfence_system();
    __syncthreads();
    if (tid == 0) {
        *p.ticket = 0u;
        if (p.work_counter) *p.work_counter = 0u;
        if (p.host_flag && !p.shard.world) st_release_sys_u64(p.host_flag, p.host_seq);
        if (p.trace) p.trace[4] = global_timer_ns();
    }
    if (p.shard.world) shard_exchange_cta(p.shard, p.out, p.k, reinterpret_cast<uint32_t *>(scratch));
    return true;
}

template <int E>
__device__ __forceinline__ void finish_u4_nominees(const ScanParams &p, WarpTopK<E> &tk) {
    __shared__ SelectScratch ss;
    __shared__ uint32_t s_cut;
    const uint32_t tid = threadIdx.x, nthr = blockDim.x;
    if (tid == 0) s_cut = WAXVS_UKEY_NONE;
    auto own_keys = [&](auto f) {
#pragma unroll
        for (int j = 0; j < E; ++j) f(tk.key[j]);
    };
    const uint64_t xa = nthr * E >= kU4CtaNominees ? block_select_kth(own_keys, kU4CtaNominees, &ss) : WAXVS_KEY_NONE;
    if (tid == 0) ss.n_sel = 0;
    __syncthreads();
    uint64_t *mine = p.nominees + static_cast<size_t>(blockIdx.x) * kU4CtaNominees;
#pragma unroll
    for (int j = 0; j < E; ++j)
        if (tk.key[j] != WAXVS_KEY_NONE && tk.key[j] <= xa) mine[atomicAdd(&ss.n_sel, 1u)] = tk.key[j];
    if ((tid & 31u) == 0 && tk.thresh != WAXVS_KEY_NONE) atomicMin(&s_cut, static_cast<uint32_t>(tk.thresh >> 32));
    __syncthreads();
    for (uint32_t i = ss.n_sel + tid; i < kU4CtaNominees; i += nthr) mine[i] = WAXVS_KEY_NONE;
    if (tid == 0) {
        uint32_t cut = s_cut;
        if (xa != WAXVS_KEY_NONE) cut = min(cut, static_cast<uint32_t>(xa >> 32));
        if (cut != WAXVS_UKEY_NONE) atomicMin(p.u4_aux, cut);
    }
}

template <int C, int R, int METRIC, int E, bool EMIT, bool SHADOW = false, bool INT8 = false, bool U4 = false>
__global__ void __launch_bounds__(512, 1) scan_tma_kernel(const __grid_constant__ ScanParams p) {
    static_assert(!SHADOW || (C > 0 && METRIC != kL2 && !EMIT), "the shadow form covers the unrolled cosine / dot shapes");
    static_assert(!INT8 || (SHADOW && R >= 4), "the int8 form is a shadow form with 16-byte scale copies");
    static_assert(!U4 || (SHADOW && !INT8 && R >= 4 && E == 4), "the 4-bit form is a shadow form with 16-byte scale copies");
    constexpr bool SCALED = INT8 || U4;
    if constexpr (!SHADOW && !EMIT && E == 1 && METRIC != kL2) {
        if (p.proof_ok) {
            const bool proven = *p.proof_ok != 0u;
            if (blockIdx.x == 0) {
                if (threadIdx.x == 0) {
                    const uint32_t n = ++p.proof_count[proven ? 0 : 1];
                    *static_cast<volatile uint32_t *>(p.proof_count_host + (proven ? 0 : 1)) = n;
                }
                if (proven && p.host_flag) {
                    for (uint32_t i = threadIdx.x; i < p.k; i += blockDim.x) p.host_out[i] = p.out[i];
                    __threadfence_system();
                    __syncthreads();
                    if (threadIdx.x == 0) st_release_sys_u64(p.host_flag, p.host_seq);
                }
            }
            if (proven) return;
        }
    }
    const int D4 = C > 0 ? 32 * C : static_cast<int>(p.dims / 4u);
    const int CN = C > 0 ? C : (D4 + 31) / 32;
    const uint32_t ROW_BYTES = C > 0 ? (U4 ? 64u : INT8 ? 128u : SHADOW ? 256u : 512u) * C : p.dims * 4u;
    const uint32_t STAGE_BYTES = ROW_BYTES * R + (SCALED ? R * 4u : 0u);
    constexpr int LANES_PER_ROW = 32 / R;

    extern __shared__ __align__(128) unsigned char smem[];
    const int warp = threadIdx.x >> 5, lane = threadIdx.x & 31, warps = blockDim.x >> 5;
    const uint32_t stages = p.stages;
    unsigned char *ring = smem + static_cast<size_t>(warp) * stages * STAGE_BYTES;
    uint64_t *bars = reinterpret_cast<uint64_t *>(smem + static_cast<size_t>(warps) * stages * STAGE_BYTES) +
                     warp * stages;
    uint64_t *lists = reinterpret_cast<uint64_t *>(smem + static_cast<size_t>(warps) * stages * STAGE_BYTES) +
                      warps * stages;
    uint32_t *stage_step = reinterpret_cast<uint32_t *>(lists + warps * 32 * E) + warp * stages;
    float4 *qs = reinterpret_cast<float4 *>(reinterpret_cast<uint32_t *>(lists + warps * 32 * E) + warps * stages + 4);

    float4 q[C > 0 ? C : 1];
    const float4 *q4 = reinterpret_cast<const float4 *>(p.query);
    const float4 *qp = reinterpret_cast<const float4 *>(p.query_inline);
    auto load_q = [&](int i) -> float4 { return q4 ? __ldg(q4 + i) : qp[i]; };
    if (C > 0) {
#pragma unroll
        for (int c = 0; c < (C > 0 ? C : 1); ++c) q[c] = load_q(lane + 32 * c);
    } else {
        qs = reinterpret_cast<float4 *>((reinterpret_cast<uintptr_t>(qs) + 15) & ~uintptr_t(15));
        for (int i = threadIdx.x; i < CN * 32; i += blockDim.x) qs[i] = (i < D4) ? load_q(i) : make_float4(0.f, 0.f, 0.f, 0.f);
        __syncthreads();
    }
    auto qchunk = [&](int c) -> float4 { return C > 0 ? q[C > 0 ? c : 0] : qs[lane + 32 * c]; };
    if constexpr (SHADOW) {
        if (p.query_store && p.query == nullptr && blockIdx.x == 0)
            for (uint32_t i = threadIdx.x; i < p.dims; i += blockDim.x) p.query_store[i] = p.query_inline[i];
    }
    constexpr int CU = U4 ? (C > 0 ? C : 1) : 1;
    constexpr int H = U4 ? R / 2 : 1;
    const int hl = lane & 15, hh = lane >> 4;
    int qlo[CU], qhi[CU], word_of[CU];
    int q_code_sum = 0;
    float s_q = 0.0f;
    if constexpr (U4) {
        float m = 0.0f;
        bool bad = false;
#pragma unroll
        for (int c = 0; c < CU; ++c) {
            bad |= !finite_f32(q[c].x) || !finite_f32(q[c].y) || !finite_f32(q[c].z) || !finite_f32(q[c].w);
            m = fmaxf(m, fmaxf(fmaxf(fabsf(q[c].x), fabsf(q[c].y)), fmaxf(fabsf(q[c].z), fabsf(q[c].w))));
        }
#pragma unroll
        for (int o = 16; o > 0; o >>= 1) m = fmaxf(m, __shfl_xor_sync(WAXVS_FULL_MASK, m, o));
        bad = __any_sync(WAXVS_FULL_MASK, bad);
        s_q = __fdiv_rn(m, 127.0f);
        const bool code_it = !bad && s_q > 0.0f && finite_f32(s_q);
        double r2 = 0.0;
#pragma unroll
        for (int c = 0; c < CU; ++c) {
            word_of[c] = hl + 16 * ((C % 2 == 0) ? (c ^ hh) : c);
            int packed[2];
#pragma unroll
            for (int half = 0; half < 2; ++half) {
                const float4 x4 = load_q(2 * word_of[c] + half);
                const float xs[4] = {x4.x, x4.y, x4.z, x4.w};
                uint32_t w = 0;
#pragma unroll
                for (int j = 0; j < 4; ++j) {
                    const int code = code_it ? max(-127, min(127, __float2int_rn(__fdiv_rn(xs[j], s_q)))) : 0;
                    w |= static_cast<uint32_t>(code & 0xFF) << (8 * j);
                    const double e = static_cast<double>(xs[j]) - static_cast<double>(s_q) * static_cast<double>(code);
                    r2 = fma(e, e, r2);
                }
                packed[half] = static_cast<int>(w);
                q_code_sum = __dp4a(packed[half], 0x01010101, q_code_sum);
            }
            qlo[c] = packed[0]; qhi[c] = packed[1];
        }
#pragma unroll
        for (int o = 8; o > 0; o >>= 1) {
            q_code_sum += __shfl_xor_sync(WAXVS_FULL_MASK, q_code_sum, o);
            r2 += __shfl_xor_sync(WAXVS_FULL_MASK, r2, o);
        }
        if (blockIdx.x == 0 && threadIdx.x == 0) {
            float rho_q = __double2float_ru(sqrt(r2) * (1.0 + 0x1p-40));
            if (bad || !finite_f32(s_q) || !finite_f32(rho_q)) rho_q = INFINITY;
            p.u4_aux[1] = __float_as_uint(rho_q);
        }
    }
    float a2 = 0.0f, sqrt_a2 = 0.0f;
    if (METRIC == kCosine && !SHADOW) {
        float s0 = 0.f, s1 = 0.f, s2 = 0.f, s3 = 0.f;
#pragma unroll
        for (int c = 0; c < CN; ++c) {
            const float4 qc = qchunk(c);
            s0 = __fmaf_rn(qc.x, qc.x, s0); s1 = __fmaf_rn(qc.y, qc.y, s1);
            s2 = __fmaf_rn(qc.z, qc.z, s2); s3 = __fmaf_rn(qc.w, qc.w, s3);
        }
        a2 = warp_butterfly_sum(__fadd_rn(__fadd_rn(s0, s1), __fadd_rn(s2, s3)));
        sqrt_a2 = __fsqrt_rn(a2);
    }

    if (p.trace && threadIdx.x == 0) atomicMin(p.trace + 0, global_timer_ns());
    const uint32_t total_warps = gridDim.x * warps;
    const uint32_t gwarp = blockIdx.x * warps + warp;
    const uint32_t n_steps = (p.n_rows + R - 1) / R;
    uint64_t policy = 0;
    if (p.use_l2_hint) policy = l2_policy_evict_first();

    auto issue = [&](uint32_t step, uint32_t s) {
        const uint32_t row0 = step * R;
        const uint32_t rows = min(static_cast<uint32_t>(R), p.n_rows - row0);
        const uint32_t bytes = rows * ROW_BYTES;
        stage_step[s] = step;
        mbar_arrive_expect_tx(&bars[s], bytes + (SCALED ? R * 4u : 0u));
        const void *src = SHADOW ? static_cast<const void *>(reinterpret_cast<const unsigned char *>(p.corpus) +
                                                             static_cast<size_t>(row0) * ROW_BYTES)
                                 : static_cast<const void *>(p.corpus + static_cast<size_t>(row0) * p.dims);
        if (p.use_l2_hint) bulk_copy_g2s_hint(ring + s * STAGE_BYTES, src, bytes, &bars[s], policy);
        else bulk_copy_g2s(ring + s * STAGE_BYTES, src, bytes, &bars[s]);
        if constexpr (SCALED) bulk_copy_g2s(ring + s * STAGE_BYTES + R * ROW_BYTES, p.row_scale + row0, R * 4u, &bars[s]);
    };

    const bool dynamic = !EMIT && p.chunk_steps > 0 && p.work_counter != nullptr;
    const uint32_t chunk = p.chunk_steps;
    uint32_t cur = gwarp, cur_end = 0, claim_l0 = 0;
    if (dynamic) {
        if (lane == 0) { cur = atomicAdd(p.work_counter, chunk); claim_l0 = atomicAdd(p.work_counter, chunk); }
        cur = __shfl_sync(WAXVS_FULL_MASK, cur, 0);
        cur_end = min(cur + chunk, n_steps);
    }
    auto next_step = [&]() -> uint32_t {
        if (!dynamic) { const uint32_t st = cur; cur = (cur < n_steps) ? cur + total_warps : cur; return st; }
        if (cur < cur_end) return cur++;
        if (cur >= n_steps) return n_steps;
        const uint32_t start = __shfl_sync(WAXVS_FULL_MASK, claim_l0, 0);
        if (lane == 0 && start < n_steps) claim_l0 = atomicAdd(p.work_counter, chunk);
        cur = start;
        cur_end = min(start + chunk, n_steps);
        if (cur >= n_steps) return n_steps;
        return cur++;
    };

    if (lane == 0) {
        for (uint32_t s = 0; s < stages; ++s) mbar_init(&bars[s], 1);
        mbar_fence_init();
    }
    __syncwarp();
    uint32_t issued = 0, consumed = 0;
    for (uint32_t s = 0; s < stages; ++s) {
        const uint32_t step = next_step();
        if (step >= n_steps) break;
        if (lane == 0) issue(step, s);
        ++issued;
    }

    WarpTopK<E> tk;
    tk.init();
    const int k = static_cast<int>(p.k);

    uint32_t s = 0, parity = 0;
    while (consumed < issued) {
        mbar_wait_parity(&bars[s], parity);
        const uint32_t step = stage_step[s];
        const float4 *tile = reinterpret_cast<const float4 *>(ring + s * STAGE_BYTES);
        const int my_in_step = U4 ? 2 * (hl / (16 / H)) + hh : lane / LANES_PER_ROW;
        const float row_s = SCALED ? reinterpret_cast<const float *>(ring + s * STAGE_BYTES + R * ROW_BYTES)[my_in_step] : 1.0f;

        float sum0[R], sum1[R];
        int isum[H] = {};
        if constexpr (U4) {
            const uint32_t *tw = reinterpret_cast<const uint32_t *>(tile) + hh * 16 * C;
#pragma unroll
            for (int j = 0; j < H; ++j) {
                int a = 0;
#pragma unroll
                for (int c = 0; c < CU; ++c) {
                    const uint32_t w = tw[j * 32 * C + word_of[c]];
                    a = __dp4a(static_cast<int>(w & 0x0F0F0F0Fu), qlo[c], a);
                    a = __dp4a(static_cast<int>((w >> 4) & 0x0F0F0F0Fu), qhi[c], a);
                }
                isum[j] = a;
            }
        } else if (C == 0) {
            float a[R][4], b[R][4];
#pragma unroll
            for (int r = 0; r < R; ++r)
#pragma unroll
                for (int j = 0; j < 4; ++j) { a[r][j] = 0.f; b[r][j] = 0.f; }
#pragma unroll (R >= 8 ? 1 : 8 / R)
            for (int c = 0; c < CN; ++c) {
                if (lane + 32 * c >= D4) break;
                const float4 qc = qchunk(c);
#pragma unroll
                for (int r = 0; r < R; ++r) {
                    const float4 v = tile[r * D4 + lane + 32 * c];
                    if (METRIC == kL2) {
                        const float dx = __fsub_rn(qc.x, v.x), dy = __fsub_rn(qc.y, v.y);
                        const float dz = __fsub_rn(qc.z, v.z), dw = __fsub_rn(qc.w, v.w);
                        a[r][0] = __fmaf_rn(dx, dx, a[r][0]); a[r][1] = __fmaf_rn(dy, dy, a[r][1]);
                        a[r][2] = __fmaf_rn(dz, dz, a[r][2]); a[r][3] = __fmaf_rn(dw, dw, a[r][3]);
                    } else {
                        a[r][0] = __fmaf_rn(qc.x, v.x, a[r][0]); a[r][1] = __fmaf_rn(qc.y, v.y, a[r][1]);
                        a[r][2] = __fmaf_rn(qc.z, v.z, a[r][2]); a[r][3] = __fmaf_rn(qc.w, v.w, a[r][3]);
                        if (METRIC == kCosine) {
                            b[r][0] = __fmaf_rn(v.x, v.x, b[r][0]); b[r][1] = __fmaf_rn(v.y, v.y, b[r][1]);
                            b[r][2] = __fmaf_rn(v.z, v.z, b[r][2]); b[r][3] = __fmaf_rn(v.w, v.w, b[r][3]);
                        }
                    }
                }
            }
#pragma unroll
            for (int r = 0; r < R; ++r) {
                sum0[r] = __fadd_rn(__fadd_rn(a[r][0], a[r][1]), __fadd_rn(a[r][2], a[r][3]));
                sum1[r] = __fadd_rn(__fadd_rn(b[r][0], b[r][1]), __fadd_rn(b[r][2], b[r][3]));
            }
        } else
#pragma unroll
        for (int r = 0; r < R; ++r) {
            float a0 = 0.f, a1 = 0.f, a2_ = 0.f, a3 = 0.f, b0 = 0.f, b1 = 0.f, b2 = 0.f, b3 = 0.f;
#pragma unroll
            for (int c = 0; c < CN; ++c) {
                if (C == 0 && lane + 32 * c >= D4) break;
                const float4 v = INT8 ? int8x4_to_float4(reinterpret_cast<const uint32_t *>(tile)[r * D4 + lane + 32 * c])
                               : SHADOW ? bf16x4_to_float4(reinterpret_cast<const uint2 *>(tile)[r * D4 + lane + 32 * c])
                                        : tile[r * D4 + lane + 32 * c];
                const float4 qc = qchunk(c);
                if (METRIC == kL2) {
                    const float dx = __fsub_rn(qc.x, v.x), dy = __fsub_rn(qc.y, v.y);
                    const float dz = __fsub_rn(qc.z, v.z), dw = __fsub_rn(qc.w, v.w);
                    a0 = __fmaf_rn(dx, dx, a0); a1 = __fmaf_rn(dy, dy, a1);
                    a2_ = __fmaf_rn(dz, dz, a2_); a3 = __fmaf_rn(dw, dw, a3);
                } else {
                    a0 = __fmaf_rn(qc.x, v.x, a0); a1 = __fmaf_rn(qc.y, v.y, a1);
                    a2_ = __fmaf_rn(qc.z, v.z, a2_); a3 = __fmaf_rn(qc.w, v.w, a3);
                    if (METRIC == kCosine && !SHADOW) {
                        b0 = __fmaf_rn(v.x, v.x, b0); b1 = __fmaf_rn(v.y, v.y, b1);
                        b2 = __fmaf_rn(v.z, v.z, b2); b3 = __fmaf_rn(v.w, v.w, b3);
                    }
                }
            }
            sum0[r] = __fadd_rn(__fadd_rn(a0, a1), __fadd_rn(a2_, a3));
            sum1[r] = __fadd_rn(__fadd_rn(b0, b1), __fadd_rn(b2, b3));
        }
        __syncwarp();
        {
            const uint32_t next = next_step();
            if (next < n_steps) {
                if (lane == 0) issue(next, s);
                ++issued;
            }
        }
        ++consumed;
        if (++s == stages) { s = 0; parity ^= 1u; }

        if constexpr (U4) half_warp_reduce_scatter<H>(isum, lane);
        else warp_reduce_scatter<R>(sum0, lane);
        if (METRIC == kCosine && !SHADOW) warp_reduce_scatter<R>(sum1, lane);

        const uint32_t my_row = step * R + my_in_step;
        float d;
        if constexpr (U4) d = -__fmul_rn(__fmul_rn(s_q, row_s), static_cast<float>(2 * isum[0] - 15 * q_code_sum));
        else if (INT8) d = -__fmul_rn(row_s, sum0[0]);
        else if (SHADOW) d = -sum0[0];
        else if (METRIC == kCosine) d = finish_cos(sum0[0], a2, sqrt_a2, sum1[0]);
        else if (METRIC == kDot) d = finish_dot(sum0[0]);
        else d = finish_l2(sum0[0]);
        if (SHADOW && !finite_f32(d)) d = -INFINITY;
        const bool leader = U4 ? (hl % (16 / H)) == 0 : (lane % LANES_PER_ROW) == 0;
        const bool ok = (my_row < p.n_rows) && (SHADOW || finite_f32(d));

        if (EMIT) {
            if (leader && my_row < p.n_rows)
                p.dist_keys[my_row] = (ok && row_allowed(p, my_row)) ? orderable_u32(d) : WAXVS_UKEY_NONE;
        } else {
            const uint64_t key = ok ? make_key(d, my_row) : WAXVS_KEY_NONE;
            const bool cand = leader && key < tk.thresh && row_allowed(p, my_row);
            uint32_t m = __ballot_sync(WAXVS_FULL_MASK, cand);
            if (E == 1) {
                while (m) {
                    const int src = __ffs(m) - 1;
                    m &= m - 1;
                    const uint64_t x = shfl_u64(key, src);
                    if (x < tk.thresh) tk.insert(x, lane, k);
                }
            } else if (m) {
                if (tk.npend + __popc(m) > 32) tk.flush(lane, k);
                while (m) {
                    const int src = __ffs(m) - 1;
                    m &= m - 1;
                    tk.park(shfl_u64(key, src), lane);
                }
            }
        }
    }

    if (p.trace && lane == 0) atomicMax(p.trace + 1, global_timer_ns());
    if (!EMIT) {
        if (E > 1) tk.flush(lane, k);
        if constexpr (U4) finish_u4_nominees<E>(p, tk);
        else if (p.tail_select) finish_topk_select<E, SHADOW>(p, tk, smem);
        else finish_topk<E, SHADOW>(p, tk, lists, warp, lane, warps);
    }
}

template <int METRIC, int E, bool EMIT>
__global__ void __launch_bounds__(256, 4) scan_ldg_kernel(const __grid_constant__ ScanParams p) {
// ... 84 lines not shown
```

wax_b200/engine.py:

```python
from __future__ import annotations

import ctypes as C
import dataclasses
import enum
import threading
from typing import Iterable, List, Optional, Sequence, Tuple

import numpy as np

from . import _lib as L


class WaxError(Exception):
    pass


class EncodingError(WaxError):
    pass


class CapacityExceeded(WaxError):
    pass


# ... 657 lines not shown
        _check(L.lib().wax_vs_shard_close(self._h))

    def shard_search(self, vector: Sequence[float], top_k: int) -> List[Tuple[int, float]]:
        q = np.ascontiguousarray(vector, dtype=np.float32).reshape(-1)
        cap = _clamp_topk(top_k)
        ids = np.empty(cap, np.uint64)
        scores = np.empty(cap, np.float32)
        n = C.c_uint32(0)
        _check(L.lib().wax_vs_shard_search(self._h, q.ctypes.data_as(C.POINTER(C.c_float)), q.size, int(top_k),
                                           ids.ctypes.data_as(C.POINTER(C.c_uint64)),
                                           scores.ctypes.data_as(C.POINTER(C.c_float)), cap, C.byref(n)))
        return [(int(ids[i]), float(scores[i])) for i in range(n.value)]

    def shard_search_filtered(self, vector: Sequence[float], top_k: int, allow: Optional[Sequence[int]] = None,
                              deny: Optional[Sequence[int]] = None) -> List[Tuple[int, float]]:
        if (allow is None) == (deny is None):
            raise ValueError("pass exactly one of allow= / deny=")
        fids = np.ascontiguousarray(allow if allow is not None else deny, dtype=np.uint64).reshape(-1)
        q = np.ascontiguousarray(vector, dtype=np.float32).reshape(-1)
        cap = _clamp_topk(top_k)
        ids = np.empty(cap, np.uint64)
        scores = np.empty(cap, np.float32)
        n = C.c_uint32(0)
        idp = fids.ctypes.data_as(C.POINTER(C.c_uint64)) if fids.size else None
        _check(L.lib().wax_vs_shard_search_filtered(self._h, q.ctypes.data_as(C.POINTER(C.c_float)), q.size, int(top_k),
                                                    idp, fids.size, 0 if allow is not None else 1,
                                                    ids.ctypes.data_as(C.POINTER(C.c_uint64)),
                                                    scores.ctypes.data_as(C.POINTER(C.c_float)), cap, C.byref(n)))
        return [(int(ids[i]), float(scores[i])) for i in range(n.value)]

    def time_shard_search(self, top_k: int, iters: int, warmup: int = 3, n_queries: int = 1, seed: int = 7):
        ms, launches = C.c_float(0), C.c_uint64(0)
        _check(L.lib().wax_vs_debug_time_shard_search(self._h, n_queries, int(top_k), seed, warmup, iters,
                                                      C.byref(ms), C.byref(launches)))
        return ms.value, launches.value

    def serialize(self) -> bytes:
        n = C.c_uint64(0)
        _check(L.lib().wax_vs_serialized_length(self._h, C.byref(n)))
        buf = bytearray(n.value)
        out = C.c_uint64(0)
        ptr = (C.c_uint8 * len(buf)).from_buffer(buf) if buf else (C.c_uint8 * 1)()
        _check(L.lib().wax_vs_serialize(self._h, ptr, len(buf), C.byref(out)))
        del ptr
        if out.value != len(buf):
            del buf[out.value:]
        return buf

    def deserialize(self, data: bytes) -> None:
        buf = np.frombuffer(data, np.uint8)
        ptr = buf.ctypes.data_as(C.POINTER(C.c_uint8)) if buf.size else C.cast(C.c_char_p(b""), C.POINTER(C.c_uint8))
        _check(L.lib().wax_vs_deserialize(self._h, ptr, buf.size))
        self._dirty = False

    def stage_for_commit(self, into) -> None:
        if not self._dirty:
            return
        into.stage_vec_index_for_next_commit(bytes=self.serialize(), vector_count=self.count,
                                             dimension=self.dimensions,
                                             similarity=self.metric.to_vec_similarity())
        self._dirty = False

    def debug_buffer_pool_stats(self) -> Tuple[int, int]:
        a, r = C.c_uint64(0), C.c_uint64(0)
        _check(L.lib().wax_vs_debug_pool_stats(self._h, C.byref(a), C.byref(r)))
        return a.value, r.value

    def fill_synthetic(self, seed: int, rows: int, first_row: int = 0, id_base: int = 0,
                       normalize: bool = True) -> None:
        _check(L.lib().wax_vs_debug_fill_synthetic(self._h, seed, first_row, rows, id_base, int(normalize)))
        self._dirty = True

    def read_rows(self, first: int, n: int) -> np.ndarray:
        out = np.empty((n, self.dimensions), np.float32)
        _check(L.lib().wax_vs_debug_read_rows(self._h, first, n, out.ctypes.data_as(C.POINTER(C.c_float))))
        return out

    def time_search(self, top_k: int, iters: int, warmup: int = 3, n_queries: int = 1, seed: int = 7):
        ms, launches = C.c_float(0), C.c_uint64(0)
        _check(L.lib().wax_vs_debug_time_search(self._h, n_queries, int(top_k), seed, warmup, iters,
                                                C.byref(ms), C.byref(launches)))
        return ms.value, launches.value

    def batch_stats(self) -> Tuple[int, int]:
        a, b = C.c_uint64(0), C.c_uint64(0)
        _check(L.lib().wax_vs_debug_batch_stats(self._h, C.byref(a), C.byref(b)))
        return a.value, b.value

    def counter(self, name: str) -> int:
        v = C.c_uint64(0)
        _check(L.lib().wax_vs_debug_counter(self._h, name.encode(), C.byref(v)))
        return v.value

    def time_search_batch(self, n_queries: int, top_k: int, iters: int, warmup: int = 2, seed: int = 7):
        ms, launches, bad = C.c_float(0), C.c_uint64(0), C.c_uint32(0)
        _check(L.lib().wax_vs_debug_time_search_batch(self._h, n_queries, int(top_k), seed, warmup, iters,
                                                      C.byref(ms), C.byref(launches), C.byref(bad)))
        return ms.value, launches.value, bad.value

    def batch_nominations(self, queries, top_k: int, allow_rows=None):
        q = np.ascontiguousarray(queries, dtype=np.float32).reshape(-1, self.dimensions)
        nq, n = q.shape[0], self.count
        scores = np.empty((nq, n), np.float32)
        ok = np.empty(nq, np.uint32)
        shape = np.zeros(7, np.uint32)
        bits = None
        if allow_rows is not None:
            mask = np.zeros(((n + 31) // 32) * 32, bool)
            mask[np.asarray(allow_rows, np.int64)] = True
            bits = (mask.reshape(-1, 32).astype(np.uint64) << np.arange(32, dtype=np.uint64)).sum(1).astype(np.uint32)
        u32 = lambda a: a.ctypes.data_as(C.POINTER(C.c_uint32))
        heaps = np.empty(0, np.uint64)
        for _ in range(2):
            rc = L.lib().wax_vs_debug_batch_nominations(
                self._h, q.ctypes.data_as(C.POINTER(C.c_float)), nq, int(top_k), None if bits is None else u32(bits),
                scores.ctypes.data_as(C.POINTER(C.c_float)), u32(ok),
                heaps.ctypes.data_as(C.POINTER(C.c_uint64)) if heaps.size else None, heaps.size, u32(shape))
            if rc != L.ERR_BUFFER or heaps.size:
                break
            heaps = np.empty(int(shape[5]) * int(shape[6]) * int(shape[4]) * 128, np.uint64)
        _check(rc)
        names = ("bf16", "ares", "pair", "stages", "kprime", "slices", "groups")
        out = {name: int(v) for name, v in zip(names, shape)}
        out.update(scores=scores, ok=ok, heaps=heaps.reshape(out["slices"] * out["groups"], out["kprime"], 128))
        return out

    def shadow_nominations(self, vector, top_k: int, allow_rows=None):
        return self._route_nominations(L.lib().wax_vs_debug_shadow_nominations, vector, top_k, allow_rows)

    def int8_nominations(self, vector, top_k: int, allow_rows=None):
        return self._route_nominations(L.lib().wax_vs_debug_int8_nominations, vector, top_k, allow_rows)

    def u4_nominations(self, vector, top_k: int, allow_rows=None):
        return self._route_nominations(L.lib().wax_vs_debug_u4_nominations, vector, top_k, allow_rows, u4=True)

    def _route_nominations(self, fn, vector, top_k: int, allow_rows, u4: bool = False):
        q = np.ascontiguousarray(vector, dtype=np.float32).reshape(self.dimensions)
        n = self.count
        k = max(1, min(int(top_k), n))
        keys = np.empty(256 * 1024 if u4 else 128, np.uint64)
        bound = np.zeros(3, np.float32)
        ok = C.c_uint32(0)
        result = (L.Candidate * k)()
        shape = np.zeros(7, np.uint32)
        bits = None
        if allow_rows is not None:
            mask = np.zeros(((n + 31) // 32) * 32, bool)
            mask[np.asarray(allow_rows, np.int64)] = True
            bits = (mask.reshape(-1, 32).astype(np.uint64) << np.arange(32, dtype=np.uint64)).sum(1).astype(np.uint32)
        u32 = lambda a: a.ctypes.data_as(C.POINTER(C.c_uint32))
        if u4:
            _check(fn(
                self._h, q.ctypes.data_as(C.POINTER(C.c_float)), int(top_k), None if bits is None else u32(bits),
                keys.ctypes.data_as(C.POINTER(C.c_uint64)), keys.size, C.byref(ok), result, u32(shape),
                bound.ctypes.data_as(C.POINTER(C.c_float))))
            keys = keys[:int(shape[4]) * 256]
        else:
            _check(fn(
                self._h, q.ctypes.data_as(C.POINTER(C.c_float)), int(top_k), None if bits is None else u32(bits),
                keys.ctypes.data_as(C.POINTER(C.c_uint64)), C.byref(ok), result, u32(shape)))
        one = np.float32(1.0)
        score = (lambda d: float(one - np.float32(d))) if self.metric is VectorMetric.cosine else (lambda d: float(-np.float32(d)))
        names = ("C", "R", "warps", "stages", "grid", "chunk_steps", "tail_select")
        out = {name: int(v) for name, v in zip(names, shape)}
        out.update(keys=keys, ok=ok.value, result=[(int(c.frame_id), score(c.distance)) for c in result if c.valid])
        if u4:
# ... 47 lines not shown
```

Measured before the change: 1499.

## Interleave per-row scales into coded shadow records for single-copy TMA stages

Stores each row's int8/4-bit scale as a trailing word inside the row's code record instead of in a separate scale array. Each pipeline stage then needs one bulk copy instead of two, and the scan kernel reads the scale from the row record. The 4-bit word indexing changes to match the new row pitch. Records no longer sit on 16-byte boundaries and the rows are padded, so bank conflicts and over-reads at the tail are possible. A debug timing entry point that splits the route into phases is also added.

```diff
diff --git a/include/wax_vs_cuda.h b/include/wax_vs_cuda.h
--- a/include/wax_vs_cuda.h
+++ b/include/wax_vs_cuda.h
@@ -237,6 +237,9 @@
 int32_t wax_vs_debug_read_u4_shadow(wax_vs_engine *engine, uint64_t first, uint64_t n, uint8_t *dst_codes,
                                     float *dst_half_steps, float *out_rho_max);
 
+int32_t wax_vs_debug_time_route_split(wax_vs_engine *engine, uint32_t n_queries, int64_t top_k, uint64_t seed,
+                                      uint32_t warmup, uint32_t iters, float *out4);
+
 int32_t wax_vs_debug_stream_read(wax_vs_engine *engine, uint32_t iters, float *out_best_ms, uint64_t *out_bytes);
 
 int32_t wax_vs_debug_set_option(wax_vs_engine *engine, const char *key, int64_t value);
diff --git a/wax_b200/_lib.py b/wax_b200/_lib.py
--- a/wax_b200/_lib.py
+++ b/wax_b200/_lib.py
@@ -124,6 +124,8 @@
                                                 C.POINTER(Candidate), _u32p, _f32p]),
     "wax_vs_debug_read_u4_shadow": (C.c_int32, [_eng, C.c_uint64, C.c_uint64, _u8p, _f32p, _f32p]),
     "wax_vs_debug_stream_read": (C.c_int32, [_eng, C.c_uint32, _f32p, _u64p]),
+    "wax_vs_debug_time_route_split": (C.c_int32, [_eng, C.c_uint32, C.c_int64, C.c_uint64, C.c_uint32, C.c_uint32,
+                                                  _f32p]),
     "wax_vs_debug_set_option": (C.c_int32, [_eng, C.c_char_p, C.c_int64]),
     "wax_vs_version": (C.c_char_p, []),
 }
diff --git a/wax_b200/csrc/waxvs_batch.cuh b/wax_b200/csrc/waxvs_batch.cuh
--- a/wax_b200/csrc/waxvs_batch.cuh
+++ b/wax_b200/csrc/waxvs_batch.cuh
@@ -247,7 +247,7 @@
 constexpr uint32_t kInt8MaxChunks = 12;
 __global__ void __launch_bounds__(256) shadow_int8_kernel(const float *__restrict__ src, const float *__restrict__ scale_in,
                                                           uint64_t n_rows, uint32_t dims, uint32_t *__restrict__ dst,
-                                                          float *__restrict__ scale, uint32_t *rho_max_bits) {
+                                                          uint32_t *rho_max_bits) {
     const int lane = threadIdx.x & 31;
     const uint64_t warps = (static_cast<uint64_t>(gridDim.x) * blockDim.x) >> 5;
     const uint32_t d4 = dims >> 2, cn = d4 / 32u;
@@ -283,12 +283,12 @@
                 const double e = static_cast<double>(xs[j]) - static_cast<double>(s) * static_cast<double>(code);
                 r2 = fma(e, e, r2);
             }
-            dst[row * d4 + lane + 32u * c] = packed;
+            dst[row * (d4 + 1u) + lane + 32u * c] = packed;
         }
         for (int o = 16; o > 0; o >>= 1) r2 += __shfl_xor_sync(WAXVS_FULL_MASK, r2, o);
         float rho = __double2float_ru(sqrt(r2) * (1.0 + 0x1p-40));
         if (bad || !finite_f32(s) || !finite_f32(rho)) rho = INFINITY;
-        if (lane == 0) scale[row] = s;
+        if (lane == 0) dst[row * (d4 + 1u) + d4] = __float_as_uint(s);
         local_max = max(local_max, __float_as_uint(rho));
     }
     if (lane == 0 && local_max) atomicMax(rho_max_bits, local_max);
@@ -296,7 +296,7 @@
 
 __global__ void __launch_bounds__(256) shadow_u4_kernel(const float *__restrict__ src, const float *__restrict__ scale_in,
                                                         uint64_t n_rows, uint32_t dims, uint32_t *__restrict__ dst,
-                                                        float *__restrict__ half_step, uint32_t *rho_max_bits) {
+                                                        uint32_t *rho_max_bits) {
     const int lane = threadIdx.x & 31;
     const uint64_t warps = (static_cast<uint64_t>(gridDim.x) * blockDim.x) >> 5;
     const uint32_t d4 = dims >> 2, cn = d4 / 32u;
@@ -333,12 +333,12 @@
                 r2 = fma(e, e, r2);
             }
             const uint32_t high = __shfl_down_sync(WAXVS_FULL_MASK, nibbles, 1);
-            if ((lane & 1) == 0) dst[row * (d4 / 2u) + (lane >> 1) + 16u * c] = nibbles | (high << 4);
+            if ((lane & 1) == 0) dst[row * (d4 / 2u + 1u) + (lane >> 1) + 16u * c] = nibbles | (high << 4);
         }
         for (int o = 16; o > 0; o >>= 1) r2 += __shfl_xor_sync(WAXVS_FULL_MASK, r2, o);
         float rho = __double2float_ru(sqrt(r2) * (1.0 + 0x1p-40));
         if (bad || !finite_f32(h) || !finite_f32(rho)) rho = INFINITY;
-        if (lane == 0) half_step[row] = h;
+        if (lane == 0) dst[row * (d4 / 2u + 1u) + d4 / 2u] = __float_as_uint(h);
         local_max = max(local_max, __float_as_uint(rho));
     }
     if (lane == 0 && local_max) atomicMax(rho_max_bits, local_max);
diff --git a/wax_b200/csrc/waxvs_engine.cu b/wax_b200/csrc/waxvs_engine.cu
--- a/wax_b200/csrc/waxvs_engine.cu
+++ b/wax_b200/csrc/waxvs_engine.cu
@@ -238,6 +238,7 @@
     uint32_t seen_failed = 0;
     bool last_u4 = false;
     DevBuf<uint32_t> d_u4_aux;
+    cudaEvent_t split_ev[2] = {nullptr, nullptr};
     ~SearchCtx() {
         if (ev0) cudaEventDestroy(ev0);
         if (ev1) cudaEventDestroy(ev1);
@@ -283,13 +284,13 @@
     struct CodedShadow {
         uint32_t bits = 8;
         DevBuf<uint32_t> codes;
-        DevBuf<float> scale;
         DevBuf<uint32_t> rho;
+        uint32_t record_words(uint32_t dims) const { return dims * bits / 32 + 1; }
         uint64_t rows = 0;
         bool valid = false, unavailable = false;
         bool coarse = false;
         float rho_max = 0.0f, eps_rel = INFINITY;
-        void release() { codes.release(); scale.release(); rows = 0; valid = false; }
+        void release() { codes.release(); rows = 0; valid = false; }
         void invalidate(uint64_t keep_prefix) {
             rows = std::min(rows, keep_prefix);
             valid = false;
@@ -785,7 +786,6 @@
     ScanParams sp = p;
     sp.corpus = u4 ? reinterpret_cast<const float *>(e->u4.codes.p)
                    : int8 ? reinterpret_cast<const float *>(e->i8.codes.p) : reinterpret_cast<const float *>(e->d_shadow.p);
-    sp.row_scale = u4 ? e->u4.scale.p : int8 ? e->i8.scale.p : nullptr;
     sp.u4_aux = u4 ? c->d_u4_aux.p : nullptr;
     sp.k = kShadowNominees;
     sp.out = nullptr; sp.host_out = nullptr; sp.host_flag = nullptr;
@@ -795,8 +795,10 @@
     sp.tail_smem_bytes = static_cast<uint32_t>(static_cast<size_t>(cfg.warps) * cfg.stages * cfg.R * e->dims *
                                                (int8 ? 1 : sizeof(__nv_bfloat16)));
     const int grid = tma_grid(e, c, cfg, sp);
-    if (u4) CUDA_TRY(launch_u4_scan(e, sp, grid, cfg, stream));
-    else if (int8) CUDA_TRY(launch_int8_scan(e, sp, grid, cfg, e->similarity, stream));
+    if (u4) {
+        CUDA_TRY(launch_u4_scan(e, sp, grid, cfg, stream));
+        if (c->split_ev[0]) CUDA_TRY(cudaEventRecord(c->split_ev[0], stream));
+    } else if (int8) CUDA_TRY(launch_int8_scan(e, sp, grid, cfg, e->similarity, stream));
     else CUDA_TRY(launch_shadow_scan(e, sp, grid, cfg, e->similarity, stream));
 
     if (u4) {
@@ -811,6 +813,7 @@
         const auto kernel = e->similarity == WAX_VS_COSINE ? shadow_rescore_kernel<kCosine> : shadow_rescore_kernel<kDot>;
         kernel<<<grid, 512, rp.tail_smem_bytes, stream>>>(rp);
         CUDA_TRY(cudaGetLastError());
+        if (c->split_ev[1]) CUDA_TRY(cudaEventRecord(c->split_ev[1], stream));
     } else {
     FinishParams fp{};
     fp.corpus = e->d_corpus; fp.queries = p.query ? p.query : c->d_queries.p;
@@ -1130,14 +1133,14 @@
     int32_t rc = ensure_norms_locked(e, stream);
     if (rc) return rc;
     if ((rc = cs.rho.ensure(1, "coded shadow bound"))) return rc;
-    const size_t words = e->dims * cs.bits / 32;
+    const size_t words = cs.record_words(e->dims);
     const uint64_t need = e->n_rows, pref = std::max<uint64_t>(e->cap_rows, e->n_rows);
-    auto scale_entries = [](uint64_t rows) { return static_cast<size_t>((rows + 15) / 16 * 16); };
-    if (cs.codes.cap < need * words || cs.scale.cap < scale_entries(need)) {
+    auto padded = [](uint64_t rows) { return static_cast<size_t>((rows + kCodedPadRows - 1) / kCodedPadRows * kCodedPadRows); };
+    if (cs.codes.cap < padded(need) * words) {
         cs.release();
         size_t free_b = 0, total_b = 0;
         uint64_t want = pref;
-        auto bytes_for = [&](uint64_t rows) { return rows * words * sizeof(uint32_t) + scale_entries(rows) * sizeof(float); };
+        auto bytes_for = [&](uint64_t rows) { return padded(rows) * words * sizeof(uint32_t); };
         const bool info = cudaMemGetInfo(&free_b, &total_b) == cudaSuccess;
         const size_t headroom = std::max<size_t>(size_t(2) << 30, total_b / 10);
         size_t reserve = 0;
@@ -1148,16 +1151,14 @@
         }
         if (info && free_b < bytes_for(want) + reserve + headroom) want = need;
         if (!info || free_b < bytes_for(want) + reserve + headroom ||
-            cudaMalloc(&cs.codes.p, want * words * sizeof(uint32_t)) != cudaSuccess ||
-            cudaMalloc(&cs.scale.p, scale_entries(want) * sizeof(float)) != cudaSuccess) {
+            cudaMalloc(&cs.codes.p, bytes_for(want)) != cudaSuccess) {
             cudaGetLastError();
             cs.release();
             cs.unavailable = true;
             return WAX_VS_OK;
         }
-        cs.codes.cap = want * words;
-        cs.scale.cap = scale_entries(want);
-        CUDA_TRY(cudaMemsetAsync(cs.scale, 0, scale_entries(want) * sizeof(float), stream));
+        cs.codes.cap = padded(want) * words;
+        CUDA_TRY(cudaMemsetAsync(cs.codes, 0, bytes_for(want), stream));
     }
     if (cs.rows > e->n_rows) cs.rows = 0;
     if (cs.rows == 0) CUDA_TRY(cudaMemsetAsync(cs.rho, 0, sizeof(uint32_t), stream));
@@ -1166,7 +1167,7 @@
         const int grid = static_cast<int>(std::min<uint64_t>(static_cast<uint64_t>(e->sm_count) * 8, (count + 7) / 8));
         (cs.bits == 4 ? shadow_u4_kernel : shadow_int8_kernel)<<<std::max(grid, 1), 256, 0, stream>>>(
             e->d_corpus + first * e->dims, e->similarity == WAX_VS_COSINE ? e->d_inv_norm + first : nullptr, count, e->dims,
-            cs.codes + first * words, cs.scale + first, cs.rho);
+            cs.codes + first * words, cs.rho);
         CUDA_TRY(cudaGetLastError());
     }
     uint32_t bits[2] = {0, 0};
@@ -4326,6 +4327,78 @@
     return WAX_VS_OK;
 }
 
+int32_t wax_vs_debug_time_route_split(wax_vs_engine *e, uint32_t n_queries, int64_t top_k, uint64_t seed, uint32_t warmup,
+                                      uint32_t iters, float *out4) {
+    if (!e || !out4) return fail(WAX_VS_ERR_NULL, "NULL argument");
+    if (n_queries == 0) n_queries = 1;
+    if (iters == 0) return fail(WAX_VS_ERR_ARGUMENT, "iters must be > 0");
+    std::shared_lock<std::shared_mutex> r(e->rw);
+    DeviceGuard g(e->device);
+    CtxLease lease(e);
+    int32_t rc = lease.acquire();
+    if (rc) return rc;
+    SearchCtx *c = lease.c;
+    const uint32_t k_eff = clamp_topk(top_k);
+    if ((rc = c->d_queries.ensure(static_cast<size_t>(n_queries) * e->dims, "query buffer")) ||
+        (rc = c->d_out.ensure(static_cast<size_t>(n_queries) * k_eff, "result buffer")))
+        return rc;
+    synth_fill_kernel<<<(n_queries + 255) / 256, 256, 0, c->stream>>>(c->d_queries, n_queries, e->dims, seed, 0, 1);
+    CUDA_TRY(cudaGetLastError());
+    if (shadow_route_applies(e)) {
+        RouteForm form;
+        if ((rc = select_route_form(e, c->stream, false, &form))) return rc;
+    }
+    struct Events {
+        cudaEvent_t ev[2] = {nullptr, nullptr};
+        ~Events() { for (cudaEvent_t x : ev) if (x) cudaEventDestroy(x); }
+    } split;
+    for (cudaEvent_t &x : split.ev) CUDA_TRY(cudaEventCreate(&x));
+    struct Unset {
+        SearchCtx *c;
+        ~Unset() { c->split_ev[0] = c->split_ev[1] = nullptr; }
+    } unset{c};
+    double sum[3] = {0, 0, 0};
+    for (uint32_t it = 0; it < warmup + iters; ++it) {
+        const uint32_t qi = it % n_queries;
+        auto u4_queries = [e] { std::lock_guard<std::mutex> pg(e->pool_mu); return e->single_u4_queries; };
+        const uint64_t u0 = u4_queries();
+        c->split_ev[0] = split.ev[0]; c->split_ev[1] = split.ev[1];
+        uint64_t launches = 0;
+        CUDA_TRY(cudaEventRecord(c->ev0, c->stream));
+        rc = enqueue_search(e, c, c->d_queries + static_cast<size_t>(qi) * e->dims, k_eff, 0,
+                            c->d_out + static_cast<size_t>(qi) * k_eff, nullptr, c->stream, &launches, nullptr, nullptr,
+                            nullptr, false, true);
+        if (rc) { cudaStreamSynchronize(c->stream); return rc; }
+        CUDA_TRY(cudaEventRecord(c->ev1, c->stream));
+        CUDA_TRY(cudaStreamSynchronize(c->stream));
+        if (u4_queries() != u0 + 1 || launches != 3)
+            return fail(WAX_VS_ERR_UNSUPPORTED, "the query did not take the 4-bit form of the route");
+        float ms[3];
+        CUDA_TRY(cudaEventElapsedTime(&ms[0], c->ev0, split.ev[0]));
+        CUDA_TRY(cudaEventElapsedTime(&ms[1], split.ev[0], split.ev[1]));
+        CUDA_TRY(cudaEventElapsedTime(&ms[2], split.ev[1], c->ev1));
+        if (it >= warmup) for (int i = 0; i < 3; ++i) sum[i] += ms[i];
+    }
+    for (int i = 0; i < 3; ++i) out4[i] = static_cast<float>(sum[i] / iters);
+    const uint64_t bytes = std::min<uint64_t>(e->n_rows * (e->dims / 2 + sizeof(float)), e->n_rows * e->dims * sizeof(float)) / 16 * 16;
+    float best = 1e30f;
+    for (int it = 0; it < 5; ++it) {
+        CUDA_TRY(cudaEventRecord(c->ev0, c->stream));
+        stream_read_kernel<<<e->sm_count * 4, 512, 0, c->stream>>>(reinterpret_cast<const uint4 *>(e->d_corpus), bytes / 16,
+                                                                     c->d_ticket + 2);
+        CUDA_TRY(cudaGetLastError());
+        CUDA_TRY(cudaEventRecord(c->ev1, c->stream));
+        CUDA_TRY(cudaStreamSynchronize(c->stream));
+        float ms = 0;
+        CUDA_TRY(cudaEventElapsedTime(&ms, c->ev0, c->ev1));
+        if (it >= 2) best = std::min(best, ms);
+    }
+    CUDA_TRY(cudaMemsetAsync(c->d_ticket, 0, 4 * sizeof(uint32_t), c->stream));
+    CUDA_TRY(cudaStreamSynchronize(c->stream));
+    out4[3] = best;
+    return WAX_VS_OK;
+}
+
 int32_t wax_vs_debug_transfer_probe(wax_vs_engine *e, uint64_t bytes, float *out7) {
     if (!e || !out7) return fail(WAX_VS_ERR_NULL, "NULL argument");
     std::unique_lock<std::shared_mutex> w(e->rw);
@@ -4634,6 +4707,16 @@
                                    keys_cap, out_bound);
 }
 
+static cudaError_t read_records(const wax_vs_engine::CodedShadow &cs, uint32_t dims, uint64_t first, uint64_t n,
+                                uint8_t *dst_codes, float *dst_scales) {
+    const size_t pitch = cs.record_words(dims) * sizeof(uint32_t), code_bytes = pitch - sizeof(float);
+    const unsigned char *src = reinterpret_cast<const unsigned char *>(cs.codes.p) + first * pitch;
+    cudaError_t err = cudaMemcpy2D(dst_codes, code_bytes, src, pitch, code_bytes, n, cudaMemcpyDeviceToHost);
+    if (err == cudaSuccess)
+        err = cudaMemcpy2D(dst_scales, sizeof(float), src + code_bytes, pitch, sizeof(float), n, cudaMemcpyDeviceToHost);
+    return err;
+}
+
 int32_t wax_vs_debug_read_u4_shadow(wax_vs_engine *e, uint64_t first, uint64_t n, uint8_t *dst_codes, float *dst_half_steps,
                                     float *out_rho_max) {
     if (!e || !dst_codes || !dst_half_steps || !out_rho_max) return fail(WAX_VS_ERR_NULL, "NULL argument");
@@ -4650,8 +4733,7 @@
     if ((rc = ensure_coded_shadow(e, e->u4, lease.c->stream, true))) return rc;
     if (!e->u4.valid) return fail(WAX_VS_ERR_UNSUPPORTED, "the 4-bit shadow does not fit in device memory");
     if (n) {
-        CUDA_TRY(cudaMemcpy(dst_codes, e->u4.codes + first * (e->dims / 8), n * e->dims / 2, cudaMemcpyDeviceToHost));
-        CUDA_TRY(cudaMemcpy(dst_half_steps, e->u4.scale + first, n * sizeof(float), cudaMemcpyDeviceToHost));
+        CUDA_TRY(read_records(e->u4, e->dims, first, n, dst_codes, dst_half_steps));
     }
     *out_rho_max = e->u4.rho_max;
     return WAX_VS_OK;
@@ -4673,8 +4755,7 @@
     if ((rc = ensure_coded_shadow(e, e->i8, lease.c->stream, true))) return rc;
     if (!e->i8.valid) return fail(WAX_VS_ERR_UNSUPPORTED, "the int8 shadow does not fit in device memory");
     if (n) {
-        CUDA_TRY(cudaMemcpy(dst_codes, e->i8.codes + first * (e->dims / 4), n * e->dims, cudaMemcpyDeviceToHost));
-        CUDA_TRY(cudaMemcpy(dst_scales, e->i8.scale + first, n * sizeof(float), cudaMemcpyDeviceToHost));
+        CUDA_TRY(read_records(e->i8, e->dims, first, n, dst_codes, dst_scales));
     }
     *out_rho_max = e->i8.rho_max;
     return WAX_VS_OK;
diff --git a/wax_b200/csrc/waxvs_scan.cuh b/wax_b200/csrc/waxvs_scan.cuh
--- a/wax_b200/csrc/waxvs_scan.cuh
+++ b/wax_b200/csrc/waxvs_scan.cuh
@@ -38,11 +38,11 @@
     const uint32_t *proof_ok;
     uint32_t *proof_count;
     uint32_t *proof_count_host;
-    const float *row_scale;
     uint32_t *u4_aux;
 };
 
 constexpr uint32_t kU4CtaNominees = 256;
+constexpr uint32_t kCodedPadRows = 16;
 
 constexpr int kNomineeStride = 128;
 
@@ -322,8 +322,8 @@
 template <int C, int R, int METRIC, int E, bool EMIT, bool SHADOW = false, bool INT8 = false, bool U4 = false>
 __global__ void __launch_bounds__(512, 1) scan_tma_kernel(const __grid_constant__ ScanParams p) {
     static_assert(!SHADOW || (C > 0 && METRIC != kL2 && !EMIT), "the shadow form covers the unrolled cosine / dot shapes");
-    static_assert(!INT8 || (SHADOW && R >= 4), "the int8 form is a shadow form with 16-byte scale copies");
-    static_assert(!U4 || (SHADOW && !INT8 && R >= 4 && E == 4), "the 4-bit form is a shadow form with 16-byte scale copies");
+    static_assert(!INT8 || (SHADOW && R >= 4 && R <= kCodedPadRows), "the int8 form is a shadow form of 16-byte steps");
+    static_assert(!U4 || (SHADOW && !INT8 && R >= 4 && R <= kCodedPadRows && E == 4), "the 4-bit form is a shadow form of 16-byte steps");
     constexpr bool SCALED = INT8 || U4;
     if constexpr (!SHADOW && !EMIT && E == 1 && METRIC != kL2) {
         if (p.proof_ok) {
@@ -345,8 +345,8 @@
     }
     const int D4 = C > 0 ? 32 * C : static_cast<int>(p.dims / 4u);
     const int CN = C > 0 ? C : (D4 + 31) / 32;
-    const uint32_t ROW_BYTES = C > 0 ? (U4 ? 64u : INT8 ? 128u : SHADOW ? 256u : 512u) * C : p.dims * 4u;
-    const uint32_t STAGE_BYTES = ROW_BYTES * R + (SCALED ? R * 4u : 0u);
+    const uint32_t ROW_BYTES = C > 0 ? (U4 ? 64u : INT8 ? 128u : SHADOW ? 256u : 512u) * C + (SCALED ? 4u : 0u) : p.dims * 4u;
+    const uint32_t STAGE_BYTES = ROW_BYTES * R;
     constexpr int LANES_PER_ROW = 32 / R;
 
     extern __shared__ __align__(128) unsigned char smem[];
@@ -399,7 +399,7 @@
         double r2 = 0.0;
 #pragma unroll
         for (int c = 0; c < CU; ++c) {
-            word_of[c] = hl + 16 * ((C % 2 == 0) ? (c ^ hh) : c);
+            word_of[c] = hh == 0 ? hl + 16 * c : (hl + 16 * c + (C % 2 == 0 ? 15 : 16 * C - 1)) % (16 * C);
             int packed[2];
 #pragma unroll
             for (int half = 0; half < 2; ++half) {
@@ -452,15 +452,14 @@
     auto issue = [&](uint32_t step, uint32_t s) {
         const uint32_t row0 = step * R;
         const uint32_t rows = min(static_cast<uint32_t>(R), p.n_rows - row0);
-        const uint32_t bytes = rows * ROW_BYTES;
+        const uint32_t bytes = (SCALED ? static_cast<uint32_t>(R) : rows) * ROW_BYTES;
         stage_step[s] = step;
-        mbar_arrive_expect_tx(&bars[s], bytes + (SCALED ? R * 4u : 0u));
+        mbar_arrive_expect_tx(&bars[s], bytes);
         const void *src = SHADOW ? static_cast<const void *>(reinterpret_cast<const unsigned char *>(p.corpus) +
                                                              static_cast<size_t>(row0) * ROW_BYTES)
                                  : static_cast<const void *>(p.corpus + static_cast<size_t>(row0) * p.dims);
         if (p.use_l2_hint) bulk_copy_g2s_hint(ring + s * STAGE_BYTES, src, bytes, &bars[s], policy);
         else bulk_copy_g2s(ring + s * STAGE_BYTES, src, bytes, &bars[s]);
-        if constexpr (SCALED) bulk_copy_g2s(ring + s * STAGE_BYTES + R * ROW_BYTES, p.row_scale + row0, R * 4u, &bars[s]);
     };
 
     const bool dynamic = !EMIT && p.chunk_steps > 0 && p.work_counter != nullptr;
@@ -506,18 +505,19 @@
         const uint32_t step = stage_step[s];
         const float4 *tile = reinterpret_cast<const float4 *>(ring + s * STAGE_BYTES);
         const int my_in_step = U4 ? 2 * (hl / (16 / H)) + hh : lane / LANES_PER_ROW;
-        const float row_s = SCALED ? reinterpret_cast<const float *>(ring + s * STAGE_BYTES + R * ROW_BYTES)[my_in_step] : 1.0f;
+        const float row_s = SCALED ? *reinterpret_cast<const float *>(ring + s * STAGE_BYTES + (my_in_step + 1) * ROW_BYTES - 4u) : 1.0f;
 
         float sum0[R], sum1[R];
         int isum[H] = {};
         if constexpr (U4) {
-            const uint32_t *tw = reinterpret_cast<const uint32_t *>(tile) + hh * 16 * C;
+            constexpr int RW = 16 * CU + 1;
+            const uint32_t *tw = reinterpret_cast<const uint32_t *>(tile) + hh * RW;
 #pragma unroll
             for (int j = 0; j < H; ++j) {
                 int a = 0;
 #pragma unroll
                 for (int c = 0; c < CU; ++c) {
-                    const uint32_t w = tw[j * 32 * C + word_of[c]];
+                    const uint32_t w = tw[j * 2 * RW + word_of[c]];
                     a = __dp4a(static_cast<int>(w & 0x0F0F0F0Fu), qlo[c], a);
                     a = __dp4a(static_cast<int>((w >> 4) & 0x0F0F0F0Fu), qhi[c], a);
                 }
@@ -563,7 +563,7 @@
 #pragma unroll
             for (int c = 0; c < CN; ++c) {
                 if (C == 0 && lane + 32 * c >= D4) break;
-                const float4 v = INT8 ? int8x4_to_float4(reinterpret_cast<const uint32_t *>(tile)[r * D4 + lane + 32 * c])
+                const float4 v = INT8 ? int8x4_to_float4(reinterpret_cast<const uint32_t *>(tile)[r * (D4 + 1) + lane + 32 * c])
                                : SHADOW ? bf16x4_to_float4(reinterpret_cast<const uint2 *>(tile)[r * D4 + lane + 32 * c])
                                         : tile[r * D4 + lane + 32 * c];
                 const float4 qc = qchunk(c);
diff --git a/wax_b200/engine.py b/wax_b200/engine.py
--- a/wax_b200/engine.py
+++ b/wax_b200/engine.py
@@ -763,6 +763,11 @@
                                                 C.byref(ms), C.byref(launches)))
         return ms.value, launches.value
 
+    def time_route_split(self, top_k: int, iters: int, warmup: int = 3, n_queries: int = 1, seed: int = 7):
+        out = (C.c_float * 4)()
+        _check(L.lib().wax_vs_debug_time_route_split(self._h, n_queries, int(top_k), seed, warmup, iters, out))
+        return tuple(float(x) for x in out)
+
     def batch_stats(self) -> Tuple[int, int]:
         a, b = C.c_uint64(0), C.c_uint64(0)
         _check(L.lib().wax_vs_debug_batch_stats(self._h, C.byref(a), C.byref(b)))
```

New measurement: 1501 (median of 6 runs). About the same (+0.1%).
